# vedrocks15/Gradient-Based-Path-Tracing

Measured on AMD Instinct MI355X. Metric: GDPT Msamples/s (base+4 offset) + Poisson ms, cbox 512x512, higher is better.
Workload: dtype f64

## Files before the change

### gradient-based-path-tracing_amd/__init__.py

```python
import ctypes as C
import os

import numpy as np

from ._ctypes_defs import *
from . import _ctypes_defs as defs

_HERE = os.path.dirname(os.path.abspath(__file__))
LIB_PATH = os.path.join(_HERE, "libgdpt.so")
_LIB = None


class GdptError(RuntimeError):
    """Raised for a non-zero status from the C ABI (the reference throws fl_exception, src/flexception.h)."""


def library_path():
    return LIB_PATH


def lib():
    global _LIB
    if _LIB is None:
        if not os.path.exists(LIB_PATH):
# ... 7 lines not shown
        L.gdpt_parse_scene.argtypes = [C.c_char_p, C.POINTER(C.POINTER(defs.GdptSceneDesc))]
        L.gdpt_parse_scene_film.argtypes = [C.c_char_p, C.c_int, C.c_int, C.POINTER(C.POINTER(defs.GdptSceneDesc))]
        L.gdpt_free_scene_desc.argtypes = [C.POINTER(defs.GdptSceneDesc)]
        L.gdpt_scene_upload.argtypes = [C.POINTER(defs.GdptSceneDesc), C.c_int, C.POINTER(vp)]
        L.gdpt_scene_free.argtypes = [vp]
        L.gdpt_scene_info.argtypes = [vp] + [C.POINTER(C.c_int32)] * 4
        L.gdpt_render.argtypes = [vp, C.POINTER(defs.GdptRenderParams), dp, dp, dp, dp, dp, C.POINTER(defs.GdptRenderStats)]
        L.gdpt_render_device.argtypes = [vp, C.POINTER(defs.GdptRenderParams), vp, vp, vp, vp, vp, vp, C.POINTER(defs.GdptRenderStats)]
        L.gdpt_path_render.argtypes = [vp, C.POINTER(defs.GdptRenderParams), dp, C.POINTER(defs.GdptRenderStats)]
        L.gdpt_path_render_device.argtypes = [vp, C.POINTER(defs.GdptRenderParams), vp, vp, C.POINTER(defs.GdptRenderStats)]
        L.gdpt_render_window_device.argtypes = [vp, C.POINTER(defs.GdptRenderParams), C.POINTER(defs.GdptSampleWindow), vp, vp, vp, vp, vp, vp,
                                                C.POINTER(defs.GdptRenderStats)]
        L.gdpt_path_render_window_device.argtypes = [vp, C.POINTER(defs.GdptRenderParams), C.POINTER(defs.GdptSampleWindow), vp, vp,
                                                     C.POINTER(defs.GdptRenderStats)]
        L.gdpt_progressive_create.argtypes = [vp, C.POINTER(defs.GdptProgressiveConfig), vp, C.POINTER(vp)]
        L.gdpt_progressive_free.argtypes = [vp]
        L.gdpt_progressive_free.restype = None
        L.gdpt_progressive_add_pass.argtypes = [vp, C.c_int, C.POINTER(defs.GdptRenderStats)]
        L.gdpt_progressive_status.argtypes = [vp, C.POINTER(defs.GdptProgressiveStatus)]
        L.gdpt_progressive_read.argtypes = [vp, C.c_int, C.POINTER(vp), C.POINTER(vp), C.POINTER(vp)]
        L.gdpt_progressive_reconstruct.argtypes = [vp, C.c_double, C.POINTER(defs.GdptReconParams), C.c_int, vp, C.POINTER(defs.GdptReconStats)]
        L.gdpt_progressive_run.argtypes = [vp, C.c_double, C.c_int, C.c_int, C.POINTER(defs.GdptProgressiveStatus)]
        L.gdpt_progressive_create_slice.argtypes = [vp, C.POINTER(defs.GdptProgressiveConfig), C.c_int, C.c_int, vp, C.POINTER(vp)]
        L.gdpt_progressive_merge.argtypes = [vp, vp]
        L.gdpt_progressive_group_create.argtypes = [C.POINTER(defs.GdptSceneDesc), C.POINTER(C.c_int32), C.c_int,
                                                    C.POINTER(defs.GdptProgressiveConfig), C.POINTER(vp)]
        L.gdpt_progressive_group_free.argtypes = [vp]
        L.gdpt_progressive_group_free.restype = None
        L.gdpt_progressive_group_run.argtypes = [vp, C.c_double, C.c_int, C.c_int, C.POINTER(defs.GdptProgressiveStatus)]
        L.gdpt_progressive_group_total.argtypes = [vp]
        L.gdpt_progressive_group_total.restype = vp
        L.gdpt_progressive_group_member_status.argtypes = [vp, C.c_int, C.POINTER(defs.GdptProgressiveStatus)]
        sst, grp = C.POINTER(defs.GdptReconSpreadStats), C.POINTER(defs.GdptGroupReconParams)
        L.gdpt_recon_spread_device.argtypes = [C.c_int, C.c_int, C.c_int, C.POINTER(vp), dp, vp, C.c_int, vp, vp, vp, sst]
        L.gdpt_recon_spread.argtypes = [C.c_int, C.c_int, C.c_int, C.POINTER(vp), dp, vp, C.c_int, vp, vp, sst]
        L.gdpt_progressive_group_reconstruct_error.argtypes = [vp, grp, C.c_int, vp, vp, vp, sst, C.POINTER(defs.GdptReconStats)]
        L.gdpt_progressive_group_run_recon.argtypes = [vp, C.c_double, C.c_int, C.c_int, C.c_int, grp,
                                                       C.POINTER(defs.GdptProgressiveStatus), sst]
        L.gdpt_assemble_device.argtypes = [C.c_int, C.c_int, vp, vp, vp, vp, vp, vp, vp, vp, vp]
        L.gdpt_poisson_solve.argtypes = [C.c_int, C.c_int, dp, dp, dp, C.c_double, dp]
        L.gdpt_poisson_solve_ex.argtypes = [C.c_int, C.c_int, dp, dp, dp, C.c_double, dp, C.c_int, C.c_double, C.c_int,
                                            C.POINTER(defs.GdptPoissonStats)]
        L.gdpt_poisson_solve_device.argtypes = [C.c_int, C.c_int, vp, vp, vp, C.c_double, vp, C.c_int, C.c_double, C.c_int,
                                                vp, C.POINTER(defs.GdptPoissonStats)]
        L.gdpt_assemble_solve_device.argtypes = [C.c_int, C.c_int, vp, vp, vp, vp, vp, vp, vp, vp, C.c_double, vp, C.c_int, C.c_double, C.c_int,
                                                 vp, C.POINTER(defs.GdptPoissonStats)]
        L.gdpt_gradient_path_render.argtypes = [vp, C.POINTER(defs.GdptRenderParams), C.c_double, dp, dp, dp, dp, dp, dp,
                                                C.POINTER(defs.GdptRenderStats), C.POINTER(defs.GdptPoissonStats)]
        L.gdpt_reconstruct.argtypes = [C.c_int, C.c_int, dp, dp, dp, C.c_double, C.POINTER(defs.GdptReconParams), dp,
                                       C.POINTER(defs.GdptReconStats)]
        L.gdpt_reconstruct_device.argtypes = [C.c_int, C.c_int, vp, vp, vp, C.c_double, C.POINTER(defs.GdptReconParams), vp, vp,
                                              C.POINTER(defs.GdptReconStats)]
        L.gdpt_gradient_path_render_recon.argtypes = [vp, C.POINTER(defs.GdptRenderParams), C.c_double, C.POINTER(defs.GdptReconParams),
                                                      dp, dp, dp, dp, dp, dp, C.POINTER(defs.GdptRenderStats), C.POINTER(defs.GdptReconStats)]
        wp, wst = C.POINTER(defs.GdptWeightedReconParams), C.POINTER(defs.GdptWeightedReconStats)
        L.gdpt_reconstruct_weighted.argtypes = [C.c_int, C.c_int, dp, dp, dp, dp, dp, dp, C.c_double, wp, dp, C.POINTER(vp), wst]
        L.gdpt_reconstruct_weighted_device.argtypes = [C.c_int, C.c_int, vp, vp, vp, vp, vp, vp, C.c_double, wp, vp, C.POINTER(vp), vp, wst]
        L.gdpt_progressive_reconstruct_weighted.argtypes = [vp, C.c_double, wp, C.c_int, vp, C.POINTER(vp), wst]
        L.gdpt_imwrite.argtypes = [C.c_char_p, C.c_int, C.c_int, dp]
        L.gdpt_imread.argtypes = [C.c_char_p, C.c_int, C.POINTER(C.c_int), C.POINTER(C.c_int), C.POINTER(dp)]
        L.gdpt_image_free.argtypes = [dp]
        L.gdpt_bvh_check.argtypes = [C.POINTER(C.c_float), C.c_int, C.POINTER(C.c_int32)]
        L.gdpt_sbvh_check.argtypes = [C.POINTER(C.c_float), C.c_int, C.c_double, C.c_int, C.POINTER(C.c_int32)]
        L.gdpt_assemble_rows_device.argtypes = [C.c_int] * 4 + [vp] * 9
        L.gdpt_band_rows.argtypes = [C.c_int, C.c_int, C.c_int, C.POINTER(C.c_int32), C.POINTER(C.c_int32)]
        L.gdpt_band_rows_weighted.argtypes = [C.c_int, C.c_int, C.c_int, C.POINTER(C.c_double), C.c_int, C.POINTER(C.c_int32), C.POINTER(C.c_int32)]
        L.gdpt_tile_row_costs.argtypes = [vp, C.c_int, C.POINTER(C.c_double), C.c_int]
        L.gdpt_poisson_forget_stream.argtypes = [vp]
        L.gdpt_band_rows_from_row_costs.argtypes = [C.c_int, C.c_int, C.c_int, C.POINTER(C.c_double), C.c_int, C.POINTER(C.c_int32), C.POINTER(C.c_int32)]
        L.gdpt_multi_rebalance.argtypes = [vp, C.POINTER(C.c_double), C.c_int]
        L.gdpt_multi_create.argtypes = [C.POINTER(defs.GdptSceneDesc), C.POINTER(defs.GdptMultiConfig), C.POINTER(vp)]
        L.gdpt_multi_free.argtypes = [vp]
        L.gdpt_multi_free.restype = None
        L.gdpt_multi_gradient_path_render.argtypes = [vp, C.POINTER(defs.GdptRenderParams), C.c_double, dp, dp, dp, dp, dp, dp,
                                                      C.POINTER(defs.GdptRenderStats), C.POINTER(defs.GdptMultiStats)]
        L.gdpt_debug_knob_set.argtypes = [C.c_char_p, C.c_double]
        L.gdpt_debug_knobs_reset.restype = None
        L.gdpt_debug_chunk_plan.argtypes = [C.c_int, C.c_int, C.c_longlong, C.c_longlong, C.POINTER(C.c_int32), C.c_int]
        L.gdpt_debug_get_stamps.argtypes = [C.POINTER(C.c_double)]
        L.gdpt_debug_get_stamps.restype = None
        L.gdpt_debug_last_route.restype = C.c_char_p
        L.gdpt_debug_overlapped_launches.argtypes = [vp]
        L.gdpt_debug_overlapped_launches.restype = C.c_longlong
        L.gdpt_debug_route_names.argtypes = [C.POINTER(C.c_char_p), C.c_int]
        _LIB = L
    return _LIB


def _check(rc):
    if rc != 0:
        raise GdptError(lib().gdpt_last_error().decode("utf-8", "replace"))


def _dp(a):
    return a.ctypes.data_as(C.POINTER(C.c_double))


class SceneDesc:

    def __init__(self, ptr):
        self.ptr = ptr

    @property
    def desc(self):
        return self.ptr.contents

    @property
    def width(self):
        return self.ptr.contents.camera.width

    @property
    def height(self):
        return self.ptr.contents.camera.height

    def close(self):
        if self.ptr:
            lib().gdpt_free_scene_desc(self.ptr)
            self.ptr = None

    def __del__(self):
        try:
            self.close()
        except Exception:
            pass


def parse_scene(filename, film=(0, 0)):
    p = C.POINTER(defs.GdptSceneDesc)()
    _check(lib().gdpt_parse_scene_film(os.fsencode(filename), int(film[0]), int(film[1]), C.byref(p)))
    return SceneDesc(p)


def _params(spp, rng_scheme, rows, max_depth_override=0, shift=0, plan_rows=0):
    p = defs.GdptRenderParams()
    p.shift_mode = int(shift)
    p.plan_rows = int(plan_rows)
    p.spp, p.rng_scheme = int(spp), int(rng_scheme)
    p.row_begin, p.row_end = int(rows[0]), int(rows[1])
    p.max_depth_override = int(max_depth_override)
    return p


class Scene:

    def __init__(self, scene_desc, device=0):
        self.desc = scene_desc
        self.width, self.height = scene_desc.width, scene_desc.height
        h = C.c_void_p()
        _check(lib().gdpt_scene_upload(scene_desc.ptr, int(device), C.byref(h)))
        self.handle = h

    def info(self):
        v = [C.c_int32() for _ in range(4)]
        _check(lib().gdpt_scene_info(self.handle, *[C.byref(x) for x in v]))
        return dict(zip(("num_nodes", "num_tris", "num_spheres", "bvh_depth"), [x.value for x in v]))

    def render(self, spp=0, rng_scheme=defs.RNG_SAMPLE, rows=(0, 0), shift=defs.SHIFT_REFERENCE, plan_rows=0):
        shape = (self.height, self.width, 3)
        bufs = {k: np.zeros(shape, dtype=np.float64) for k in ("img", "cx0", "cy0", "cx1", "cy1")}
        st = defs.GdptRenderStats()
        p = _params(spp, rng_scheme, rows, shift=shift, plan_rows=plan_rows)
        _check(lib().gdpt_render(self.handle, C.byref(p), _dp(bufs["img"]), _dp(bufs["cx0"]), _dp(bufs["cy0"]),
                                 _dp(bufs["cx1"]), _dp(bufs["cy1"]), C.byref(st)))
        return bufs, st

    def render_device(self, ptrs, spp=0, rng_scheme=defs.RNG_SAMPLE, rows=(0, 0), stream=None, want_stats=False,
                      shift=defs.SHIFT_REFERENCE, plan_rows=0, window=None):
        st = defs.GdptRenderStats() if want_stats else None
        p = _params(spp, rng_scheme, rows, shift=shift, plan_rows=plan_rows)
        tail = [C.c_void_p(int(x)) for x in ptrs] + [C.c_void_p(int(stream) if stream else 0), C.byref(st) if st is not None else None]
        if window is None:
            _check(lib().gdpt_render_device(self.handle, C.byref(p), *tail))
        else:
            win = defs.GdptSampleWindow(int(window[0]), int(window[1]))
            _check(lib().gdpt_render_window_device(self.handle, C.byref(p), C.byref(win), *tail))
        return st

    def path_render(self, spp=0, rng_scheme=defs.RNG_SAMPLE, rows=(0, 0), want_counts=False):
        img = np.zeros((self.height, self.width, 3), dtype=np.float64)
        st = defs.GdptRenderStats()
        if want_counts:
            st.nodes_visited = 2 ** 64 - 1
        p = _params(spp, rng_scheme, rows)
        _check(lib().gdpt_path_render(self.handle, C.byref(p), _dp(img), C.byref(st)))
        return img, st

    def path_render_device(self, ptr, spp=0, rng_scheme=defs.RNG_SAMPLE, rows=(0, 0), stream=None, window=None, want_stats=False):
        st = defs.GdptRenderStats() if want_stats else None
        p = _params(spp, rng_scheme, rows)
        tail = [C.c_void_p(int(ptr)), C.c_void_p(int(stream) if stream else 0), C.byref(st) if st is not None else None]
        if window is None:
            _check(lib().gdpt_path_render_device(self.handle, C.byref(p), *tail))
        else:
            win = defs.GdptSampleWindow(int(window[0]), int(window[1]))
            _check(lib().gdpt_path_render_window_device(self.handle, C.byref(p), C.byref(win), *tail))
        return st

    def gradient_path_render(self, spp=0, rng_scheme=defs.RNG_SAMPLE, alpha=0.04, return_buffers=False,
                             shift=defs.SHIFT_REFERENCE, plan_rows=0, reconstruct=None):
        shape = (self.height, self.width, 3)
        out = np.zeros(shape, dtype=np.float64)
        bufs = {k: np.zeros(shape, dtype=np.float64) for k in ("img", "cx0", "cy0", "cx1", "cy1")}
        rs = defs.GdptRenderStats()
        p = _params(spp, rng_scheme, (0, 0), shift=shift, plan_rows=plan_rows)
        raw = [_dp(bufs[k]) for k in ("img", "cx0", "cy0", "cx1", "cy1")]
        if reconstruct is None:
            ps = defs.GdptPoissonStats()
            _check(lib().gdpt_gradient_path_render(self.handle, C.byref(p), float(alpha), _dp(out), *raw, C.byref(rs), C.byref(ps)))
        else:
            ps = defs.GdptReconStats()
            _check(lib().gdpt_gradient_path_render_recon(self.handle, C.byref(p), float(alpha), C.byref(reconstruct), _dp(out), *raw,
                                                         C.byref(rs), C.byref(ps)))
        return (out, bufs, rs, ps) if return_buffers else out

    def tile_row_costs(self, spp=1):
        T = (self.height + 15) // 16
        buf = (C.c_double * T)()
        _check(lib().gdpt_tile_row_costs(self.handle, int(spp), buf, T))
        return [float(x) for x in buf]

    def overlapped_launches(self):
        return int(lib().gdpt_debug_overlapped_launches(self.handle))

    def close(self):
        if getattr(self, "handle", None):
            lib().gdpt_scene_free(self.handle)
            self.handle = None

    def __del__(self):
        try:
            self.close()
        except Exception:
            pass


BUFFERS = ("img", "cx0", "cy0", "cx1", "cy1")


class Progressive:

    def __init__(self, scene, budget_spp, shift=defs.SHIFT_REFERENCE, path=False, stream=None, max_depth_override=0, slice=None):
        self.scene = scene
        self._owned = True
        self.path = bool(path)
        self.names = BUFFERS[:1] if self.path else BUFFERS
        self.shape = (scene.height, scene.width, 3)
        cfg = defs.GdptProgressiveConfig(defs.PROGRESSIVE_PATH if self.path else defs.PROGRESSIVE_GRADPATH, int(shift), int(budget_spp),
                                         int(max_depth_override))
        h = C.c_void_p()
        if slice is None:
            _check(lib().gdpt_progressive_create(scene.handle, C.byref(cfg), C.c_void_p(int(stream) if stream else 0), C.byref(h)))
        else:
            _check(lib().gdpt_progressive_create_slice(scene.handle, C.byref(cfg), int(slice[0]), int(slice[1]),
                                                       C.c_void_p(int(stream) if stream else 0), C.byref(h)))
        self.handle = h

    @classmethod
    def _view(cls, owner, handle, shape, path):
        self = cls.__new__(cls)
        self.scene, self._owned = owner, False
        self.path = bool(path)
        self.names = BUFFERS[:1] if self.path else BUFFERS
        self.shape = shape
        self.handle = C.c_void_p(handle)
        return self

    def merge(self, other):
        _check(lib().gdpt_progressive_merge(self.handle, other.handle))
        return self.status()

    def add_pass(self, spp):
        st = defs.GdptRenderStats()
        _check(lib().gdpt_progressive_add_pass(self.handle, int(spp), C.byref(st)))
        return st

    @staticmethod
    def _status_dict(st):
        return dict(passes=st.passes, spp=st.spp_done, budget_spp=st.budget_spp, error=st.error_estimate,
                    pixels_left_out=st.pixels_left_out, fold_ms=st.fold_ms, stop_reason=defs.STOP_NAMES[st.stop_reason], totals=st.totals)

    def status(self):
        st = defs.GdptProgressiveStatus()
        _check(lib().gdpt_progressive_status(self.handle, C.byref(st)))
        return self._status_dict(st)

    def read(self, variances=True):
        variances = bool(variances) and self.status()["passes"] >= 2
        means = {k: np.empty(self.shape, dtype=np.float64) for k in self.names}
        vars_ = {k: np.empty(self.shape, dtype=np.float64) for k in self.names} if variances else None
        asm = {k: np.empty(self.shape, dtype=np.float64) for k in ("c", "cx", "cy")} if variances and not self.path else None

        def table(d, keys):
            arr = (C.c_void_p * len(keys))()
            for i, k in enumerate(keys):
                arr[i] = d[k].ctypes.data if d is not None and k in d else None
            return arr
        _check(lib().gdpt_progressive_read(self.handle, 0, table(means, BUFFERS), table(vars_, BUFFERS), table(asm, ("c", "cx", "cy"))))
        return means, vars_, asm

    def read_device(self, mean_ptrs=None, var_ptrs=None, assembled_var_ptrs=None):
        def table(ptrs, n):
            arr = (C.c_void_p * n)()
            for i in range(n):
# ... 346 lines not shown
def shape_triangles(scene_desc):
    d = scene_desc.desc
    out = []
    for i in range(d.num_shapes):
        sh = d.shapes[i]
        if sh.num_triangles <= 0:
            continue
        pos = np.ctypeslib.as_array(sh.positions, shape=(sh.num_vertices, 3)).astype(np.float32)
        idx = np.ctypeslib.as_array(sh.indices, shape=(sh.num_triangles, 3))
        out.append(pos[idx])
    return np.concatenate(out, axis=0) if out else np.zeros((0, 3, 3), np.float32)


def shape_triangle_bounds(scene_desc):
    d = scene_desc.desc
    out = []
    for i in range(d.num_shapes):
        sh = d.shapes[i]
        if sh.num_triangles <= 0:
            continue
        pos = np.ctypeslib.as_array(sh.positions, shape=(sh.num_vertices, 3)).astype(np.float32)
        idx = np.ctypeslib.as_array(sh.indices, shape=(sh.num_triangles, 3))
        tri = pos[idx]
        out.append(np.concatenate([tri.min(axis=1), tri.max(axis=1)], axis=1))
    return np.concatenate(out, axis=0) if out else np.zeros((0, 6), np.float32)


class debug_knobs:

    def __init__(self, **knobs):
        self.knobs = knobs

    def __enter__(self):
        for k, v in self.knobs.items():
            _check(lib().gdpt_debug_knob_set(k.encode(), float(v)))
        return self

    def __exit__(self, *exc):
        lib().gdpt_debug_knobs_reset()
        return False

    @staticmethod
    def set(**knobs):
        for k, v in knobs.items():
            _check(lib().gdpt_debug_knob_set(k.encode(), float(v)))

    @staticmethod
    def reset():
        lib().gdpt_debug_knobs_reset()

    @staticmethod
    def chunk_plan(spp, film_pixels, resident_lanes=256 * 2 * 256, force_log2k=-1):
        buf = (C.c_int32 * 80)()
        n = lib().gdpt_debug_chunk_plan(int(spp), int(force_log2k), int(film_pixels), int(resident_lanes), buf, 80)
        if n < 0:
            raise GdptError("gdpt_debug_chunk_plan: capacity")
        return list(buf)[:n + 1]

    @staticmethod
    def stamps():
        v = (C.c_double * 16)()
        lib().gdpt_debug_get_stamps(v)
        d = dict(zip(("loop_head", "trace", "vertex", "consume", "bsdf", "finish", "camera", "wave_steps", "publish", "take", "item"), list(v)))
        d["busy_us"] = (v[13] - v[12]) / 100.0
        d["drain_us"] = (v[14] - v[13]) / 100.0
        return d

    @staticmethod
    def last_route():
        return lib().gdpt_debug_last_route().decode()

    @staticmethod
    def route_names():
        n = lib().gdpt_debug_route_names(None, 0)
        buf = (C.c_char_p * n)()
        if lib().gdpt_debug_route_names(buf, n) != n:
            raise GdptError("gdpt_debug_route_names: capacity")
        return [x.decode() for x in buf]

    @staticmethod
    def from_env(environ=None):
        environ = os.environ if environ is None else environ
        names = ("force_eager", "log2k", "keep_frac", "search_frac", "blocks_per_cu", "no_lds_scene", "lds_wide",
                 "no_twosided_machine", "presplit", "presplit_floor", "bvh_leaf_max", "bvh_leaf_factor", "sbvh", "sbvh_alpha", "plan_rounds", "plan_shrink", "plan_digits", "bvh_collapse_dp", "stamps", "wavefront", "wf_slots", "wf_sort", "multi_fail_band", "multi_fail_stage", "dct_bk", "dct_bm", "full_material_switch", "no_plain_kernel", "replay_per_step", "no_render_overlap")
        lib().gdpt_debug_knobs_reset()
        for n in names:
            v = environ.get("GDPT_" + n.upper())
            if v is not None:
                _check(lib().gdpt_debug_knob_set(n.encode(), float(v)))


def build_arch():
    return lib().gdpt_build_arch().decode()
```

### gradient-based-path-tracing_amd/csrc/capi_host.cpp

```cpp
#include "../../include/gdpt.h"
#include "../../include/gdpt_debug.h"
#include "capi_common.h"
#include "host/bvh.h"
#include "host/image_io.h"
#include "host/scene_loader.h"

#include <cmath>
#include <cstdlib>
#include <cstring>
#include <vector>
#include <algorithm>
#include <map>
#include <mutex>
#include <string>

namespace gdpt {
static thread_local std::string g_last_error;
void set_last_error(const std::string &msg) { g_last_error = msg; }
}

namespace gdpt {
namespace {
std::mutex g_knob_mu;
std::map<std::string, double> g_knobs;
const char *const kKnobNames[] = {"force_eager", "log2k", "keep_frac", "search_frac", "blocks_per_cu", "no_lds_scene", "lds_wide",
                                  "no_twosided_machine", "presplit", "presplit_floor", "bvh_leaf_max", "bvh_leaf_factor", "sbvh", "sbvh_alpha", "plan_rounds", "plan_shrink", "plan_digits", "bvh_collapse_dp", "stamps", "wavefront", "wf_slots", "wf_sort", "multi_fail_band", "multi_fail_stage", "dct_bk", "dct_bm", "full_material_switch", "no_plain_kernel", "replay_per_step", "no_render_overlap"};
double g_stamps[16] = {0};
}
void debug_store_stamps(const unsigned long long *v, int n) {
    std::lock_guard<std::mutex> lk(g_knob_mu);
    for (int i = 0; i < 16; i++) g_stamps[i] = i < n ? (double)v[i] : 0.0;
}
double debug_knob(const char *name, double def) {
    std::lock_guard<std::mutex> lk(g_knob_mu);
    if (g_knobs.empty()) return def;
    auto it = g_knobs.find(name);
    return it == g_knobs.end() ? def : it->second;
}
}

namespace {
std::mutex g_mu;
std::map<GdptSceneDesc *, std::unique_ptr<gdpt::HostScene>> g_descs;
}

extern "C" {

const char *gdpt_last_error(void) { return gdpt::g_last_error.c_str(); }

int gdpt_debug_knob_set(const char *name, double value) {
    return gdpt::guarded([&]() {
        if (!name) throw std::runtime_error("gdpt_debug_knob_set: null name");
        bool known = false;
        for (const char *k : gdpt::kKnobNames) if (std::strcmp(k, name) == 0) known = true;
        if (!known) throw std::runtime_error(std::string("gdpt_debug_knob_set: unknown knob '") + name + "'");
        std::lock_guard<std::mutex> lk(gdpt::g_knob_mu);
        gdpt::g_knobs[name] = value;
    });
}
void gdpt_debug_get_stamps(double out[16]) {
    std::lock_guard<std::mutex> lk(gdpt::g_knob_mu);
    for (int i = 0; i < 16; i++) out[i] = gdpt::g_stamps[i];
}
void gdpt_debug_knobs_reset(void) {
    std::lock_guard<std::mutex> lk(gdpt::g_knob_mu);
    gdpt::g_knobs.clear();
}

int gdpt_parse_scene(const char *xml_path, GdptSceneDesc **out_desc) { return gdpt_parse_scene_film(xml_path, 0, 0, out_desc); }

int gdpt_parse_scene_film(const char *xml_path, int film_width, int film_height, GdptSceneDesc **out_desc) {
    return gdpt::guarded([&]() {
        if (!xml_path || !out_desc) throw std::runtime_error("gdpt_parse_scene: null argument");
        if (film_width < 0 || film_height < 0 || film_width > 65536 || film_height > 65536) throw std::runtime_error("gdpt_parse_scene_film: bad film extent");
        std::unique_ptr<gdpt::HostScene> hs = gdpt::load_scene_xml(xml_path, film_width, film_height);
        GdptSceneDesc *d = &hs->desc;
        std::lock_guard<std::mutex> lk(g_mu);
        g_descs[d] = std::move(hs);
        *out_desc = d;
    });
}

void gdpt_free_scene_desc(GdptSceneDesc *desc) {
    std::lock_guard<std::mutex> lk(g_mu);
    g_descs.erase(desc);
}

int gdpt_imwrite(const char *filename, int width, int height, const double *rgb) {
    return gdpt::guarded([&]() {
        if (!filename || !rgb || width <= 0 || height <= 0) throw std::runtime_error("gdpt_imwrite: bad argument");
        gdpt::write_image(filename, width, height, rgb);
    });
}

int gdpt_imread(const char *filename, int channels, int *width, int *height, double **texels) {
    return gdpt::guarded([&]() {
        if (!filename || !width || !height || !texels || (channels != 1 && channels != 3)) throw std::runtime_error("gdpt_imread: bad argument");
        std::vector<double> t;
        gdpt::load_texture_file(filename, channels, width, height, &t);
        double *out = (double *)std::malloc(t.size() * sizeof(double));
        if (!out) throw std::runtime_error("gdpt_imread: out of memory");
        std::memcpy(out, t.data(), t.size() * sizeof(double));
        *texels = out;
    });
}

void gdpt_image_free(double *texels) { std::free(texels); }

int gdpt_sbvh_check(const float *tri_verts9, int n, double budget, int samples_per_tri, int32_t stats[8]) {
// ... 235 lines not shown
```

### gradient-based-path-tracing_amd/csrc/device_scene.h

```cpp
#pragma once
#include <stdint.h>

#define GDPT_BVH_MAX_DEPTH 32
#define GDPT_LEAF_MAX_PRIMS 4
#define GDPT_SPHERE_FLAG 0x80000000u
#ifndef GDPT_HBM_BVH8
#define GDPT_HBM_BVH8 0
#endif
#define GDPT_STACK_OVERFLOW 64
#ifndef GDPT_BVH8_SORT
#define GDPT_BVH8_SORT 1
#endif
#ifndef GDPT_SPEC_LEAF
#define GDPT_SPEC_LEAF 0
#endif
#define GDPT_CHILD_EMPTY INT32_MIN

struct DevBvhNode {
    float lmin[3], lmax[3];
    float rmin[3], rmax[3];
    int32_t left, right;
    int32_t pad[2];
};

struct DevBvh4Node {
    float lo[3][4];
    float hi[3][4];
    int32_t child[4];
    int32_t pad[4];
};

struct DevBvh8Node {
    int32_t child[8];
    uint8_t qlo[3][8];
    uint8_t qhi[3][8];
    float org[3];
    float scale[3];
    int32_t pad[6];
};

struct DevBvh4QNode {
    float org[3];
    float scale[3];
    uint8_t qlo[3][4];
    uint8_t qhi[3][4];
    int32_t child[4];
};
#ifndef GDPT_HBM_Q4
#define GDPT_HBM_Q4 1
#endif

struct DevPrim {
    float v0[3], e1[3], e2[3];
    uint32_t gid;
    uint32_t pad[2];
};

struct DevTriShade {
    double n[3][3];
    double uv[3][2];
    double dpdu[3], dpdv[3];
    double gn[3];
    double inv_uv_size;
    int32_t shape_id, prim_id, material_id, light_id;
    int32_t has_normals, has_uvs;
    int32_t flat_frame, pad;
};

struct DevSphere {
    double center[3];
    double radius;
    int32_t shape_id, material_id, light_id, pad;
};

struct DevLight {
    double intensity[3];
    double area;
    int32_t is_sphere;
    int32_t sphere_index;
    int32_t tri_first;
    int32_t tri_count;
    int32_t cdf_first;
    int32_t has_normals;
};

struct DevImage {
    int32_t channels, num_levels;
    int32_t width[8], height[8];
    int64_t offset[8];
};

struct DevCamera {
    double sample_to_cam[16];
    double cam_to_world[16];
    double org[3];
    int32_t width, height;
    int32_t filter_type;
    int32_t pow2_film;
    double filter_param;
    double inv_width, inv_height;
};

struct DevSceneView {
    DevCamera cam;
    const DevBvhNode *nodes;
    const DevBvh4Node *nodes4;
    const DevBvh8Node *nodes8;
    const DevBvh4QNode *nodes4q;
    const DevPrim *prims;
    const DevTriShade *tris;
    const DevSphere *spheres;
    const struct GdptMaterial *materials;
    const double *light_intensity;
    const DevImage *images;
    const double *texels;
    const DevLight *lights;
    const double *light_pmf, *light_cdf;
    const double *light_tri_cdf;
    const double *light_tri_pos;
    const double *light_tri_nrm;
    int32_t has_envmap, env_light_id, env_image_id, env_pad;
    int32_t env_w, env_h;
    double env_scale;
    double env_to_world[16], env_to_local[16];
    const double *env_cdf_rows, *env_pdf_rows, *env_cdf_marginals, *env_pdf_marginals;
    int32_t num_nodes, num_nodes4, num_nodes8, num_prims, num_tris, num_spheres;
    int32_t num_materials, num_lights, num_images;
    int32_t max_depth, rr_depth;
    int32_t all_textures_constant;
    double isect_eps;
};
```

### gradient-based-path-tracing_amd/csrc/hip/capi_device.hip

```cpp
#include "../../../include/gdpt.h"
#include "../capi_common.h"
#include "../device_scene.h"
#include "../host/bvh.h"
#include "../host/tri_precompute.h"
#include "poisson_kernels.h"
#include "recon_l1.h"
#include "recon_weighted.h"
#include "render_kernels.h"
#include "scene_internal.h"

#include <hip/hip_runtime.h>

#include <algorithm>
#include <cmath>
#include <cstdlib>
#include <cstring>
#include <limits>
#include <memory>
#include <string>
#include <vector>

namespace {

using gdpt::ck;
// ... 54 lines not shown
            for (int k = 0; k < 3; k++) { float p = (float)sh.positions[3 * i + k]; lb[k] = std::min(lb[k], p); ub[k] = std::max(ub[k], p); }
        for (int t = 0; t < sh.num_triangles; t++) {
            DevTriShade ts{};
            DevPrim pr{};
            gdpt::PrimBounds pb;
            float v[3][3];
            double pos64[3][3];
            for (int k = 0; k < 3; k++) { pb.bmin[k] = std::numeric_limits<float>::infinity(); pb.bmax[k] = -pb.bmin[k]; }
            for (int i = 0; i < 3; i++) {
                int vi = sh.indices[3 * t + i];
                if (vi < 0 || vi >= sh.num_vertices) throw std::runtime_error("gdpt_scene_upload: mesh index out of range");
                for (int k = 0; k < 3; k++) {
                    pos64[i][k] = sh.positions[3 * vi + k];
                    v[i][k] = (float)sh.positions[3 * vi + k];
                    pb.bmin[k] = std::min(pb.bmin[k], v[i][k]); pb.bmax[k] = std::max(pb.bmax[k], v[i][k]);
                    if (sh.normals) ts.n[i][k] = sh.normals[3 * vi + k];
                }
                if (sh.uvs) { ts.uv[i][0] = sh.uvs[2 * vi]; ts.uv[i][1] = sh.uvs[2 * vi + 1]; }
            }
            if (!sh.uvs) {
                ts.uv[0][0] = 0; ts.uv[0][1] = 0; ts.uv[1][0] = 1; ts.uv[1][1] = 0; ts.uv[2][0] = 1; ts.uv[2][1] = 1;
            }
            ts.shape_id = s; ts.prim_id = t; ts.material_id = sh.material_id; ts.light_id = sh.area_light_id;
            ts.has_normals = sh.normals != nullptr; ts.has_uvs = sh.uvs != nullptr;
            for (int k = 0; k < 3; k++) { pr.v0[k] = v[0][k]; pr.e1[k] = v[1][k] - v[0][k]; pr.e2[k] = v[2][k] - v[0][k]; }
            for (int i = 0; i < 3; i++) for (int k = 0; k < 3; k++) tri_verts.push_back(v[i][k]);
            gdpt::precompute_tri_constants(pos64, pr.e1, pr.e2, &ts);
            pr.gid = (uint32_t)tris.size();
            tris.push_back(ts); prim_in.push_back(pr); bounds.push_back(pb);
        }
    }
    if (tris.size() >= (size_t)GDPT_SPHERE_FLAG / 8) throw std::runtime_error("gdpt_scene_upload: too many triangles");
    for (int s = 0; s < desc->num_shapes; s++) {
        const GdptShape &sh = desc->shapes[s];
        if (sh.type != GDPT_SHAPE_SPHERE) continue;
        DevSphere sp{};
        DevPrim pr{};
        gdpt::PrimBounds pb;
        for (int k = 0; k < 3; k++) {
            sp.center[k] = sh.center[k];
            lb[k] = std::min(lb[k], (float)(sh.center[k] - sh.radius)); ub[k] = std::max(ub[k], (float)(sh.center[k] + sh.radius));
            pb.bmin[k] = std::nextafterf((float)(sh.center[k] - sh.radius), -std::numeric_limits<float>::infinity());
            pb.bmax[k] = std::nextafterf((float)(sh.center[k] + sh.radius), std::numeric_limits<float>::infinity());
        }
        sp.radius = sh.radius; sp.shape_id = s; sp.material_id = sh.material_id; sp.light_id = sh.area_light_id;
        pr.gid = GDPT_SPHERE_FLAG | (uint32_t)spheres.size();
        spheres.push_back(sp); prim_in.push_back(pr); bounds.push_back(pb);
    }

    std::vector<gdpt::PrimBounds> refs;
    std::vector<uint32_t> ref_prim;
    {
        double budget = tris.size() >= 4096 ? kPresplitBudget : 0.0;
        budget = gdpt::debug_knob("presplit", budget);
        gdpt::presplit_triangles(bounds, tri_verts, budget, &refs, &ref_prim);
    }
    const double sbvh_budget = gdpt::debug_knob("sbvh", tris.size() >= 4096 ? kSbvhBudget : 0.0);
    gdpt::BvhBuildResult bvh = sbvh_budget > 0 ? gdpt::build_sbvh(bounds, tri_verts, sbvh_budget, &ref_prim) : gdpt::build_bvh(refs);
    {
        float ext = 0.f;
        for (int k = 0; k < 3; k++) if (ub[k] >= lb[k]) ext = std::max(ext, std::max(std::fabs(ub[k]), std::fabs(lb[k])));
        for (auto &sp : spheres) for (int k = 0; k < 3; k++) ext = std::max(ext, (float)(std::fabs(sp.center[k]) + sp.radius));
        {
            const double *m = cam.cam_to_world;
            for (int k = 0; k < 3; k++) ext = std::max(ext, (float)std::fabs(m[4 * k + 3] / m[15]) * 1.0000002f);
        }
        const float pad = ext * 1e-6f + 1e-30f;
        for (auto &n : bvh.nodes)
            for (int k = 0; k < 3; k++) {
                if (n.lmin[k] <= n.lmax[k]) { n.lmin[k] -= pad; n.lmax[k] += pad; }
                if (n.rmin[k] <= n.rmax[k]) { n.rmin[k] -= pad; n.rmax[k] += pad; }
            }
    }
    gdpt::WideBvh wide = gdpt::collapse_for_traversal(bvh.nodes, GDPT_HBM_BVH8 != 0);
    if (wide.stack_need > GDPT_BVH_MAX_DEPTH) throw std::runtime_error("gdpt_scene_upload: BVH deeper than the traversal stack (builder bug)");
    if (wide.stack_need8 > GDPT_BVH_MAX_DEPTH + GDPT_STACK_OVERFLOW) throw std::runtime_error("gdpt_scene_upload: BVH8 deeper than the traversal stack (builder bug)");
    static_assert(sizeof(DevBvh8Node) == 128 && sizeof(DevBvh4Node) == 128, "wide BVH nodes are one 128-byte line");
    const std::vector<DevBvh4Node> &nodes4 = wide.nodes;
    sc->wide_stack_need = wide.stack_need;
    sc->wide8_stack_need = wide.stack_need8;
    std::vector<DevPrim> prims(bvh.order.size());
    for (size_t i = 0; i < bvh.order.size(); i++) prims[i] = prim_in[ref_prim[bvh.order[i]]];
    sc->bvh_depth = bvh.depth;
    if (bvh.depth > GDPT_BVH_MAX_DEPTH) throw std::runtime_error("gdpt_scene_upload: BVH deeper than the traversal stack (builder bug)");

    std::vector<DevImage> images;
    std::vector<double> texels;
    for (int i = 0; i < desc->num_images; i++) {
        const GdptImage &im = desc->images[i];
        if (im.width <= 0 || im.height <= 0 || (im.channels != 1 && im.channels != 3) || !im.texels)
            throw std::runtime_error("gdpt_scene_upload: bad image");
        DevImage di{};
        di.channels = im.channels;
        int size = std::max(im.width, im.height);
        int num_levels = std::min((int)std::ceil(std::log2((double)size) + 1), 8);
        di.num_levels = num_levels;
        int pw = im.width, ph = im.height;
        size_t prev_off = texels.size();
        di.width[0] = pw; di.height[0] = ph; di.offset[0] = (int64_t)prev_off;
        texels.insert(texels.end(), im.texels, im.texels + (size_t)pw * ph * im.channels);
        for (int l = 1; l < num_levels; l++) {
            int nw = std::max(pw / 2, 1), nh = std::max(ph / 2, 1);
            size_t off = texels.size();
            texels.resize(off + (size_t)nw * nh * im.channels);
            auto P = [&](int x, int y, int c) { x = std::min(x, pw - 1); y = std::min(y, ph - 1); return texels[prev_off + ((size_t)y * pw + x) * im.channels + c]; };
            for (int y = 0; y < nh; y++) for (int x = 0; x < nw; x++) for (int c = 0; c < im.channels; c++)
                texels[off + ((size_t)y * nw + x) * im.channels + c] =
                    (P(2 * x, 2 * y, c) + P(2 * x + 1, 2 * y, c) + P(2 * x, 2 * y + 1, c) + P(2 * x + 1, 2 * y + 1, c)) / 4.0;
            di.width[l] = nw; di.height[l] = nh; di.offset[l] = (int64_t)off;
            prev_off = off; pw = nw; ph = nh;
        }
        images.push_back(di);
    }

    std::vector<GdptMaterial> materials(desc->materials, desc->materials + desc->num_materials);
    std::vector<double> light_intensity;
    for (int l = 0; l < desc->num_lights; l++) for (int k = 0; k < 3; k++) light_intensity.push_back(desc->lights[l].intensity[k]);

    int env_power_slot = -1;
    std::vector<double> light_power;
    std::vector<DevLight> dlights;
    std::vector<double> light_pmf, light_cdf, light_tri_cdf, light_tri_pos, light_tri_nrm;
    auto table_1d = [](const std::vector<double> &f, std::vector<double> &pmf, std::vector<double> &cdf) {
        pmf = f;
        cdf.assign(f.size() + 1, 0.0);
        for (size_t i = 0; i < f.size(); i++) cdf[i + 1] = cdf[i] + pmf[i];
        const double total = cdf.back();
        if (total > 0) { for (size_t i = 0; i < pmf.size(); i++) { pmf[i] /= total; cdf[i] /= total; } }
        else {
            for (size_t i = 0; i < pmf.size(); i++) { pmf[i] = 1.0 / (double)pmf.size(); cdf[i] = (double)i / (double)pmf.size(); }
            cdf.back() = 1;
        }
    };
    {
        std::vector<int> sphere_index_of_shape((size_t)desc->num_shapes, -1);
        { int k = 0; for (int s = 0; s < desc->num_shapes; s++) if (desc->shapes[s].type == GDPT_SHAPE_SPHERE) sphere_index_of_shape[(size_t)s] = k++; }
        std::vector<double> power;
        for (int l = 0; l < desc->num_lights; l++) {
            const GdptLight &lt = desc->lights[l];
            if (lt.shape_id < 0 && desc->has_envmap && l == desc->envmap.light_id) {
                dlights.push_back(DevLight{});
                power.push_back(0.0);
                continue;
            }
            if (lt.shape_id < 0 || lt.shape_id >= desc->num_shapes) throw std::runtime_error("gdpt_scene_upload: light without a shape");
            const GdptShape &sh = desc->shapes[lt.shape_id];
            DevLight dl{};
            for (int k = 0; k < 3; k++) dl.intensity[k] = lt.intensity[k];
            if (sh.type == GDPT_SHAPE_SPHERE) {
                dl.is_sphere = 1; dl.sphere_index = sphere_index_of_shape[(size_t)lt.shape_id];
                dl.area = 4 * 3.14159265358979323846 * sh.radius * sh.radius;
            } else {
                dl.tri_first = (int)(light_tri_pos.size() / 9); dl.tri_count = sh.num_triangles;
                dl.cdf_first = (int)light_tri_cdf.size(); dl.has_normals = sh.normals ? 1 : 0;
                std::vector<double> areas((size_t)sh.num_triangles), pmf, cdf;
                double total = 0;
                for (int t = 0; t < sh.num_triangles; t++) {
                    const int *ix = sh.indices + 3 * t;
                    double p[3][3];
                    for (int i = 0; i < 3; i++) for (int k = 0; k < 3; k++) { p[i][k] = sh.positions[3 * ix[i] + k]; light_tri_pos.push_back(p[i][k]); }
                    for (int i = 0; i < 3; i++) for (int k = 0; k < 3; k++) light_tri_nrm.push_back(sh.normals ? sh.normals[3 * ix[i] + k] : 0.0);
                    const double e1[3] = {p[1][0] - p[0][0], p[1][1] - p[0][1], p[1][2] - p[0][2]}, e2[3] = {p[2][0] - p[0][0], p[2][1] - p[0][1], p[2][2] - p[0][2]};
                    const double cx = e1[1] * e2[2] - e1[2] * e2[1], cy = e1[2] * e2[0] - e1[0] * e2[2], cz = e1[0] * e2[1] - e1[1] * e2[0];
                    areas[(size_t)t] = std::sqrt(cx * cx + cy * cy + cz * cz) / 2;
                    total += areas[(size_t)t];
                }
// ... 160 lines not shown

Band resolve_spp(const GdptScene *sc, const GdptRenderParams *p, int scene_spp, const char *what, const GdptSampleWindow *win = nullptr) {
    Band b = resolve(sc, p);
    if (b.spp <= 0) b.spp = scene_spp;
    if (b.spp <= 0) throw std::runtime_error(std::string(what) + ": samples per pixel must be > 0");
    b.stream_spp = b.spp; b.first_sample = 0;
    if (win) {
        if (b.rng == GDPT_RNG_TILE) throw std::runtime_error(std::string(what) + ": GDPT_RNG_TILE has one stream per tile and no sample window (use GDPT_RNG_SAMPLE)");
        if (win->stream_spp <= 0 || win->first_sample < 0 || (long long)win->first_sample + b.spp > (long long)win->stream_spp)
            throw std::runtime_error(std::string(what) + ": sample window [first_sample, first_sample + spp) must lie inside [0, stream_spp)");
        if ((unsigned long long)sc->view.cam.width * (unsigned long long)sc->view.cam.height > (~0ull >> 1) / (unsigned long long)win->stream_spp)
            throw std::runtime_error(std::string(what) + ": width * height * stream_spp does not fit 63 bits");
        b.stream_spp = win->stream_spp; b.first_sample = win->first_sample;
    }
    return b;
}

struct ScratchClaim { GdptLaunchScratch *set = nullptr; bool record_release = true; };

bool is_capturing(hipStream_t stream) {
    hipStreamCaptureStatus st = hipStreamCaptureStatusNone;
    if (hipStreamIsCapturing(stream, &st) != hipSuccess) { (void)hipGetLastError(); return true; }
    return st != hipStreamCaptureStatusNone;
}

void join_scratch(GdptScene *sc) {
    sc->join();
    for (auto &ss : sc->scratch) if (ss.used) ck(hipEventSynchronize(ss.released), "hipEventSynchronize(launch scratch)");
}

GdptLaunchScratch &claim_scratch(GdptScene *sc, bool overlap, bool capturing, size_t need, hipStream_t stream) {
    const int k = overlap ? (int)(sc->overlapped & 1) : 0;
    GdptLaunchScratch &ss = sc->scratch[k];
    const hipEvent_t entry = sc->ev_entry[sc->calls & 1], prev_entry = sc->calls ? (hipEvent_t)sc->ev_entry[(sc->calls + 1) & 1] : nullptr;
    if (!capturing) { ck(hipEventRecord(entry, stream), "hipEventRecord(entry)"); sc->calls++; }
    if (capturing) {
        hipStreamCaptureMode mode = hipStreamCaptureModeRelaxed;
        ck(hipThreadExchangeStreamCaptureMode(&mode), "hipThreadExchangeStreamCaptureMode");
        try { join_scratch(sc); } catch (...) { (void)hipThreadExchangeStreamCaptureMode(&mode); throw; }
        ck(hipThreadExchangeStreamCaptureMode(&mode), "hipThreadExchangeStreamCaptureMode");
    }
    if (!ss.counters) ss.counters.alloc(1, "hipMalloc(counters)");
    if (!ss.queue) ss.queue.alloc(1, "hipMalloc(queue)");
    if (need > ss.partials.size()) {
        if (ss.partials) {
            if (!capturing) join_scratch(sc);
            sc->need_fence = true;
        }
        ss.partials.alloc(need, "hipMalloc(work-item partials)");
    }
    if (!overlap) {
        if (!capturing) {
            sc->join();
            if (ss.used) ck(hipStreamWaitEvent(stream, ss.released, 0), "hipStreamWaitEvent(launch scratch)");
        }
    } else {
        if (sc->have_caller && stream != sc->last_caller) {
            for (auto &o : sc->scratch) ck(hipStreamWaitEvent(stream, o.rendered, 0), "hipStreamWaitEvent(render stream)");
            sc->need_fence = true;
        }
        if (sc->need_fence || !prev_entry) {
            for (auto &st : sc->render_stream) ck(hipStreamWaitEvent(st, entry, 0), "hipStreamWaitEvent(fence)");
            sc->need_fence = false;
        } else
            ck(hipStreamWaitEvent(sc->render_stream[k], prev_entry, 0), "hipStreamWaitEvent(previous call)");
        if (ss.used) ck(hipStreamWaitEvent(sc->render_stream[k], ss.released, 0), "hipStreamWaitEvent(launch scratch)");
    }
    sc->have_caller = true; sc->last_caller = stream;
    return ss;
}

gdpt::RenderLaunch begin_launch(GdptScene *sc, const Band &b, bool path, int take_pct, hipStream_t stream, const GdptRenderStats *stats, ScratchClaim *claim) {
    auto knob = [](const char *name, int def) { return gdpt::debug_knob_int(name, def); };
    const DevSceneView &v = sc->view;
    gdpt::RouteInputs in{};
    in.path = path; in.rng_scheme = b.rng; in.shift_mode = b.shift; in.max_depth = b.max_depth; in.rr_depth = v.rr_depth;
    in.one_sided = sc->one_sided; in.has_rough = sc->has_rough; in.lambert_only = sc->lambert_only; in.material_mask = sc->material_mask;
    in.has_spheres = v.num_spheres != 0; in.const_textures = v.all_textures_constant != 0; in.has_envmap = v.has_envmap != 0;
    in.fits_lds = gdpt::scene_fits_lds(v.num_nodes, v.num_prims, v.num_tris, v.num_materials, v.num_lights, sc->bvh_depth);
    in.fits_lds_wide = gdpt::scene_fits_lds_wide(v.num_nodes4, v.num_prims, v.num_tris, v.num_materials, v.num_lights, sc->wide_stack_need);
    in.force_eager = knob("force_eager", 0) != 0; in.no_lds_scene = knob("no_lds_scene", 0) != 0; in.lds_wide = knob("lds_wide", 1) != 0;
    in.no_twosided_machine = knob("no_twosided_machine", 0) != 0; in.wavefront = knob("wavefront", kWavefrontDefault) != 0;
    in.stamps = knob("stamps", 0) != 0; in.no_plain_kernel = knob("no_plain_kernel", 0) != 0;
    in.full_material_switch = knob("full_material_switch", 0) != 0;
    gdpt::RenderLaunch rl{};
    rl.route = gdpt::choose_route(in);
    rl.spp = b.spp; rl.stream_spp = b.stream_spp; rl.first_sample = b.first_sample; rl.row_begin = b.row_begin; rl.row_end = b.row_end; rl.max_depth = b.max_depth;
    rl.count_traversal = stats && stats->nodes_visited == ~0ull;
    rl.force_log2k = knob("log2k", -1);
    rl.thresh_a = knob("keep_frac", -1); rl.thresh_c = knob("search_frac", -1);
    rl.num_cus = sc->num_cus; rl.blocks_per_cu = knob("blocks_per_cu", 0);
    const bool capturing = is_capturing(stream);
    const bool overlap = !stats && gdpt::can_overlap(rl.route) && !capturing && knob("no_render_overlap", 0) == 0;
    size_t need = 0;
    if (gdpt::is_persistent(rl.route)) {
        rl.plan = gdpt::make_chunk_plan(b.spp, rl.force_log2k, (long long)v.cam.width * b.plan_rows, gdpt::resident_lanes(rl), take_pct);
        need = (size_t)16 * (size_t)gdpt::band_slots(v.cam.width, b.row_end - b.row_begin) * (size_t)rl.plan.n;
    }
    GdptLaunchScratch &ss = claim_scratch(sc, overlap, capturing, need, stream);
    rl.counters = ss.counters; sc->d_counters = ss.counters;
    if (gdpt::is_persistent(rl.route)) { rl.partials = ss.partials; rl.queue_head = ss.queue; }
    if (overlap) { rl.kernel_stream = sc->render_stream[sc->overlapped & 1]; rl.kernel_done = ss.rendered; }
    claim->set = &ss; claim->record_release = !capturing;
    return rl;
}

void run_launch(GdptScene *sc, const gdpt::RenderLaunch &rl, const ScratchClaim &claim, const Band &b, hipStream_t stream, GdptRenderStats *stats) {
    const bool stamped = gdpt::is_stamped(rl.route);
    const hipStream_t ks = rl.kernel_stream ? rl.kernel_stream : stream;
    if (rl.kernel_stream) sc->in_flight = true;
    ck(hipMemsetAsync(rl.counters, 0, sizeof(gdpt::RenderCounters), ks), "hipMemsetAsync(counters)");
    if (stamped) ck(hipMemsetAsync(&rl.counters->stamps[12], 0xFF, 2 * sizeof(unsigned long long), ks), "hipMemsetAsync(stamps)");
    if (stats) ck(hipEventRecord(sc->ev0, stream), "hipEventRecord");
    gdpt::launch_render(sc->view, rl, stream);
    if (rl.kernel_stream) sc->overlapped++;
    if (claim.record_release) { ck(hipEventRecord(claim.set->released, stream), "hipEventRecord(launch scratch)"); claim.set->used = true; }
    if (!stats) return;
    ck(hipEventRecord(sc->ev1, stream), "hipEventRecord");
    ck(hipMemcpyAsync(sc->h_counters, rl.counters, sizeof(gdpt::RenderCounters), hipMemcpyDeviceToHost, stream), "hipMemcpyAsync(counters)");
    ck(hipStreamSynchronize(stream), "hipStreamSynchronize(render)");
    float ms = 0;
    ck(hipEventElapsedTime(&ms, sc->ev0, sc->ev1), "hipEventElapsedTime");
    const gdpt::RenderCounters &c = *sc->h_counters;
    std::memset(stats, 0, sizeof(*stats));
    stats->samples = (uint64_t)sc->view.cam.width * (uint64_t)(b.row_end - b.row_begin) * (uint64_t)b.spp;
    stats->rays = c.rays; stats->bounces = c.bounces; stats->nonfinite_samples = c.nonfinite;
    stats->nodes_visited = c.nodes; stats->tris_tested = c.prims;
    stats->render_ms = ms;
    if (!gdpt::is_path(rl.route)) {
        stats->wave_node_trips = c.wave_node_trips; stats->wave_leaf_trips = c.wave_leaf_trips;
        stats->wave_steps = c.wave_steps; stats->lane_steps = c.lane_steps;
    }
    if (stamped) gdpt::debug_store_stamps(c.stamps, 16);
    stats->node_bytes = gdpt::walks_bvh2(rl.route) ? sizeof(DevBvhNode) : sizeof(DevBvh4Node);
}

}

namespace gdpt {
void render_device_impl(GdptScene *sc, const GdptRenderParams *params, int scene_spp,
                        double *img, double *cx0, double *cy0, double *cx1, double *cy1,
                        hipStream_t stream, GdptRenderStats *stats, const GdptSampleWindow *window) {
    reset_route();
    ck(hipSetDevice(sc->device), "hipSetDevice");
    const Band b = resolve_spp(sc, params, scene_spp, "gdpt_render", window);
    if (!img || !cx0 || !cy0 || !cx1 || !cy1) throw std::runtime_error("gdpt_render: null output buffer");
    ScratchClaim claim;
    RenderLaunch rl = begin_launch(sc, b, false, sc->plan_take_pct, stream, stats, &claim);
    rl.img = img; rl.cx0 = cx0; rl.cy0 = cy0; rl.cx1 = cx1; rl.cy1 = cy1;
    rl.wide_stack_need = GDPT_HBM_BVH8 ? std::min(sc->wide8_stack_need, GDPT_BVH_MAX_DEPTH) : sc->wide_stack_need;
    rl.replay_per_step = debug_knob_int("replay_per_step", 0);
    const long long items = band_slots(sc->view.cam.width, b.row_end - b.row_begin) * rl.plan.n;
    if (needs_bounce_log(rl.route)) {
        sc->d_bounce_log.grow(twosided_log_bytes(persistent_blocks(rl, items)), stream, "hipMalloc(bounce log)");
        rl.bounce_log = sc->d_bounce_log; rl.bounce_log_bytes = sc->d_bounce_log.size();
    }
    if (is_wavefront(rl.route)) {
        int slots = wf_slot_count(items);
        { const int forced = debug_knob_int("wf_slots", 0); if (forced > 0) slots = std::min(slots, (forced + 255) / 256 * 256); }
        sc->d_wf_state.grow((size_t)slots * wf_words(), stream, "hipMalloc(wavefront state)");
        sc->d_wf_live.grow((size_t)slots, stream, "hipMalloc(wavefront live list)");
        sc->d_wf_aux.grow(wf_aux_bytes(slots), stream, "hipMalloc(wavefront ray / hit records)");
        if (!sc->d_wf_counters) sc->d_wf_counters.alloc((size_t)3 * wf_max_generations(), "hipMalloc(wavefront counters)");
        if (!sc->h_wf_word) sc->h_wf_word.alloc(1, "hipHostMalloc(wavefront)");
        if (!sc->wf_event) sc->wf_event.create(hipEventDisableTiming);
        rl.wf_aux = sc->d_wf_aux; rl.wf_sort = debug_knob_int("wf_sort", 1);
        for (int k = 0; k < 6; k++) rl.wf_bounds[k] = sc->bounds[k];
        rl.wf_state = sc->d_wf_state; rl.wf_live = sc->d_wf_live; rl.wf_counters = sc->d_wf_counters; rl.wf_host = sc->h_wf_word;
        rl.wf_event = sc->wf_event; rl.wf_slots = slots;
// ... 17 lines not shown
    rl.img = img;
    run_launch(sc, rl, claim, b, stream, stats);
}

gdpt::ReconL1Params resolve_recon(const GdptReconParams &in) {
    if (in.norm != GDPT_RECON_L1) throw std::runtime_error("gdpt_reconstruct: unknown norm (GDPT_RECON_L2 | GDPT_RECON_L1)");
    for (double v : {in.eps_init, in.eps_decay, in.eps_floor, in.cg_tol})
        if (!std::isfinite(v) || v < 0) throw std::runtime_error("gdpt_reconstruct: eps_init, eps_decay, eps_floor and cg_tol must be finite and >= 0 (0 = default)");
    if (in.eps_decay > 1.0) throw std::runtime_error("gdpt_reconstruct: eps_decay must lie in (0, 1]");
    gdpt::ReconL1Params p;
    p.irls_iters = in.irls_iters == 0 ? 20 : std::max(in.irls_iters, 0);
    p.cg_max_iters = in.cg_max_iters > 0 ? in.cg_max_iters : 1000;
    p.eps_init = in.eps_init > 0 ? in.eps_init : 0.05;
    p.eps_decay = in.eps_decay > 0 ? in.eps_decay : 0.5;
    p.eps_floor = in.eps_floor > 0 ? in.eps_floor : 1e-3;
    p.cg_tol = in.cg_tol > 0 ? in.cg_tol : 1e-6;
    return p;
}
using Planes = std::vector<gdpt::DeviceBuffer<double>>;
template <class F>
void on_device_planes(std::initializer_list<const double *> in, int width, int height, double *out, const char *what, F &&run) {
    const size_t elems = (size_t)width * height * 3, bytes = elems * sizeof(double);
    Planes d(in.size() + 1);
    for (auto &b : d) b.alloc(elems, what);
    size_t k = 0;
    for (const double *h : in) ck(hipMemcpy(d[k++], h, bytes, hipMemcpyHostToDevice), "hipMemcpy");
    run(d);
    ck(hipMemcpy(out, d.back(), bytes, hipMemcpyDeviceToHost), "hipMemcpy");
}

void fill_poisson_stats(GdptPoissonStats *s, const gdpt::PoissonResult &r) {
    if (!s) return;
    s->iterations = r.iterations; s->solver = r.solver; s->rel_residual = r.rel_residual; s->solve_ms = r.solve_ms;
}
void fill_recon_stats(GdptReconStats *s, const gdpt::ReconL1Result &r) {
    if (!s) return;
    s->norm = GDPT_RECON_L1; s->irls_rounds = r.irls_rounds; s->cg_iters_total = r.cg_iters_total; s->cg_iters_last = r.cg_iters_last;
    s->energy_first = r.energy_first; s->energy_last = r.energy_last; s->rel_residual_last = r.rel_residual_last; s->solve_ms = r.solve_ms;
}
void fill_recon_stats_l2(GdptReconStats *s, double solve_ms) {
    if (!s) return;
    *s = GdptReconStats{};
    s->norm = GDPT_RECON_L2; s->solve_ms = solve_ms;
}

gdpt::ReconL1Params resolve_weighted(const GdptWeightedReconParams *in, double *conf_floor, int *norm) {
    GdptReconParams rp = in ? in->recon : GdptReconParams{};
    *norm = rp.norm;
    if (rp.norm != GDPT_RECON_L2 && rp.norm != GDPT_RECON_L1) throw std::runtime_error("gdpt_reconstruct_weighted: unknown norm (GDPT_RECON_L2 | GDPT_RECON_L1)");
    rp.norm = GDPT_RECON_L1;
    gdpt::ReconL1Params p = resolve_recon(rp);
    if (*norm == GDPT_RECON_L2) p.irls_iters = 0;
    const double d = in ? in->conf_floor : 0.0;
    if (!std::isfinite(d) || d < 0) throw std::runtime_error("gdpt_reconstruct_weighted: conf_floor must be finite and > 0 (0 = default 0.05)");
    *conf_floor = d > 0 ? d : 0.05;
    return p;
}
void fill_weighted_stats(GdptWeightedReconStats *s, int norm, const gdpt::ReconWeightedResult &r) {
    if (!s) return;
    *s = GdptWeightedReconStats{};
    fill_recon_stats(&s->recon, r.recon);
    s->recon.norm = norm;
    s->scale_data = r.scale_data; s->scale_grad = r.scale_grad; s->rows_dropped = r.rows_dropped; s->pixels_isolated = r.pixels_isolated;
}

}

extern "C" {

#ifndef GDPT_BUILD_ARCH
#error "GDPT_BUILD_ARCH must name the --offload-arch the kernels were compiled for (csrc/Makefile passes it)"
#endif
const char *gdpt_build_arch(void) { return GDPT_BUILD_ARCH; }

int gdpt_debug_chunk_plan(int spp, int force_log2k, long long film_pixels, long long resident_lanes, int32_t *begin, int capacity) {
    const gdpt::ChunkPlan p = gdpt::make_chunk_plan(spp, force_log2k, film_pixels, resident_lanes);
    if (!begin || capacity < p.n + 1) return -1;
    for (int c = 0; c <= p.n; c++) begin[c] = p.begin[c];
    return p.n;
}

const char *gdpt_debug_last_route(void) { return gdpt::last_route(); }
long long gdpt_debug_overlapped_launches(const GdptScene *scene) { return scene ? (long long)scene->overlapped : -1; }
int gdpt_debug_route_names(const char **out, int capacity) { return gdpt::route_names(out, capacity); }

int gdpt_scene_upload(const GdptSceneDesc *desc, int device, GdptScene **out_scene) {
    return gdpt::guarded([&]() {
        if (!out_scene) throw std::runtime_error("gdpt_scene_upload: null output");
        std::unique_ptr<GdptScene> sc(new GdptScene());
        build_scene(desc, device, sc.get());
        sc->scene_spp = desc->samples_per_pixel;
        *out_scene = sc.release();
    });
}

void gdpt_scene_free(GdptScene *scene) {
    if (!scene) return;
    delete scene;
}

int gdpt_scene_info(const GdptScene *scene, int32_t *num_nodes, int32_t *num_tris, int32_t *num_spheres, int32_t *bvh_depth) {
    return gdpt::guarded([&]() {
        if (!scene) throw std::runtime_error("null scene handle");
        if (num_nodes) *num_nodes = scene->view.num_nodes;
        if (num_tris) *num_tris = scene->view.num_tris;
        if (num_spheres) *num_spheres = scene->view.num_spheres;
        if (bvh_depth) *bvh_depth = scene->bvh_depth;
    });
}

int gdpt_render_device(GdptScene *scene, const GdptRenderParams *params,
                       double *d_img, double *d_cx0, double *d_cy0, double *d_cx1, double *d_cy1,
                       void *stream, GdptRenderStats *stats) {
    return gdpt::guarded([&]() {
        if (!scene) throw std::runtime_error("null scene handle");
        render_device_impl(scene, params, scene->scene_spp, d_img, d_cx0, d_cy0, d_cx1, d_cy1, (hipStream_t)stream, stats);
    });
}

int gdpt_render(GdptScene *scene, const GdptRenderParams *params,
                double *img, double *cx0, double *cy0, double *cx1, double *cy1, GdptRenderStats *stats) {
    return gdpt::guarded([&]() {
        if (!scene) throw std::runtime_error("null scene handle");
        if (!img || !cx0 || !cy0 || !cx1 || !cy1) throw std::runtime_error("gdpt_render: null output buffer");
        ck(hipSetDevice(scene->device), "hipSetDevice");
        size_t elems = (size_t)scene->view.cam.width * scene->view.cam.height * 3;
        scene->ensure_buffers(elems);
        Band b = resolve(scene, params);
        double *host[5] = {img, cx0, cy0, cx1, cy1};
        bool partial = (b.row_begin != 0 || b.row_end != scene->view.cam.height);
        if (partial) for (int k = 0; k < 5; k++) ck(hipMemcpy(scene->d_buf[k], host[k], elems * sizeof(double), hipMemcpyHostToDevice), "hipMemcpy(H2D)");
        GdptRenderStats local{};
        render_device_impl(scene, params, scene->scene_spp, scene->d_buf[0], scene->d_buf[1], scene->d_buf[2], scene->d_buf[3], scene->d_buf[4],
                           nullptr, stats ? stats : &local);
        for (int k = 0; k < 5; k++) ck(hipMemcpy(host[k], scene->d_buf[k], elems * sizeof(double), hipMemcpyDeviceToHost), "hipMemcpy(D2H)");
    });
}

int gdpt_tile_row_costs(GdptScene *scene, int spp, double *cost, int capacity) {
    return gdpt::guarded([&]() {
        if (!scene || !cost) throw std::runtime_error("gdpt_tile_row_costs: null argument");
        const int H = scene->view.cam.height, T = (H + 15) / 16;
        if (capacity < T) throw std::runtime_error("gdpt_tile_row_costs: capacity < ceil(height / 16)");
        ck(hipSetDevice(scene->device), "hipSetDevice");
        scene->ensure_buffers((size_t)scene->view.cam.width * H * 3);
        for (int t = 0; t < T; t++) {
            GdptRenderParams p{};
            p.spp = spp > 0 ? spp : 1; p.rng_scheme = GDPT_RNG_SAMPLE; p.row_begin = t * 16; p.row_end = std::min(H, t * 16 + 16);
            GdptRenderStats st{};
            render_device_impl(scene, &p, scene->scene_spp, scene->d_buf[0], scene->d_buf[1], scene->d_buf[2], scene->d_buf[3], scene->d_buf[4], nullptr, &st);
            cost[t] = (double)st.rays;
        }
    });
}

int gdpt_path_render_device(GdptScene *scene, const GdptRenderParams *params, double *d_img, void *stream, GdptRenderStats *stats) {
    return gdpt::guarded([&]() {
        if (!scene) throw std::runtime_error("null scene handle");
        path_render_device_impl(scene, params, d_img, (hipStream_t)stream, stats, nullptr);
    });
}

int gdpt_render_window_device(GdptScene *scene, const GdptRenderParams *params, const GdptSampleWindow *window,
                              double *d_img, double *d_cx0, double *d_cy0, double *d_cx1, double *d_cy1,
                              void *stream, GdptRenderStats *stats) {
    if (!window) return gdpt_render_device(scene, params, d_img, d_cx0, d_cy0, d_cx1, d_cy1, stream, stats);
// ... 217 lines not shown
```

### gradient-based-path-tracing_amd/csrc/hip/render_device.h

```cpp
#pragma once
#include "render_kernels.h"
#include "device_trace.h"

namespace gd {

constexpr int kBlock = 256;
constexpr int kLdsSceneBytes = 20 * 1024;
constexpr int kLdsSceneLevels = 12;

struct LaneCounters { unsigned rays, bounces, nonfinite; };

enum { SEG_QUEUE = 0, SEG_TRACE = 1, SEG_VERTEX = 2, SEG_CONSUME = 3, SEG_BSDF = 4, SEG_FINISH = 5, SEG_CAMERA = 6, SEG_STEPS = 7, SEG_PUBLISH = 8, SEG_TAKE = 9, SEG_ITEM = 10, SEG_COUNT = 12, SEG_T_START = 12, SEG_T_DRY = 13, SEG_T_END = 14, SEG_SLOTS = 16 };
template <bool ON> struct Stamps {
    unsigned long long *slot;
    GD void start(unsigned long long *wave_row) {
        if (ON) { slot = wave_row; if ((threadIdx.x & 63) == 0) { for (int i = 0; i < SEG_COUNT; i++) slot[i] = 0; slot[SEG_COUNT] = __builtin_amdgcn_s_memtime(); } }
    }
    GD void mark(int seg) {
        if (ON) {
            __builtin_amdgcn_sched_barrier(0);
            const unsigned long long t = __builtin_amdgcn_s_memtime();
            __builtin_amdgcn_s_waitcnt(0xC07F);
            if ((int)(threadIdx.x & 63) == __ffsll((unsigned long long)__ballot(1)) - 1) { slot[seg] += t - slot[SEG_COUNT]; slot[SEG_COUNT] = t; }
            __builtin_amdgcn_sched_barrier(0);
        }
    }
    GD void tick(int seg) { if (ON) { if ((int)(threadIdx.x & 63) == __ffsll((unsigned long long)__ballot(1)) - 1) slot[seg] += 1; } }
    GD unsigned long long get(int seg) const { return ON ? slot[seg] : 0ull; }
};
struct Accum { D3 r, dx0, dy0, dx1, dy1; };

struct KernelArgs {
    int spp, log2k, tile_w, tile_h, tiles_x;
    int row_begin, row_end, max_depth;
    int thresh_a, thresh_c;
    int count;
    int stream_spp, first_sample;
    int stack_levels;
    int replay_per_step;
    int num_chunks;
    long long num_slots;
    long long num_items;
    double *partials;
    int chunk_begin[gdpt::kMaxChunks + 1];
    unsigned long long *queue_head;
    double *img, *cx0, *cy0, *cx1, *cy1;
    gdpt::RenderCounters *counters;
};

GD bool loop_allows(int max_depth, int num_vertices) { return max_depth == -1 || num_vertices <= max_depth + 1; }

struct AccReg {
    Accum a;
    GD void init() { a.r = a.dx0 = a.dy0 = a.dx1 = a.dy1 = splat(0); }
    GD void add(int which, D3 v) {
        if (which == 0) a.r = a.r + v; else if (which == 1) a.dx0 = a.dx0 + v; else if (which == 2) a.dy0 = a.dy0 + v;
        else if (which == 3) a.dx1 = a.dx1 + v; else a.dy1 = a.dy1 + v;
    }
    GD Accum result() { return a; }
};
struct AccLds {
    double *slot;
    int stride;
    GD void init() { for (int c = 0; c < 15; c++) slot[c * stride] = 0.0; }
    GD void add(int which, D3 v) {
        double *p = slot + which * 3 * stride;
        __hip_atomic_fetch_add(p, v.x, __ATOMIC_RELAXED, __HIP_MEMORY_SCOPE_WORKGROUP);
        __hip_atomic_fetch_add(p + stride, v.y, __ATOMIC_RELAXED, __HIP_MEMORY_SCOPE_WORKGROUP);
        __hip_atomic_fetch_add(p + 2 * stride, v.z, __ATOMIC_RELAXED, __HIP_MEMORY_SCOPE_WORKGROUP);
    }
    GD Accum result() {
        Accum a;
        a.r = mk(slot[0], slot[stride], slot[2 * stride]);
        a.dx0 = mk(slot[3 * stride], slot[4 * stride], slot[5 * stride]);
        a.dy0 = mk(slot[6 * stride], slot[7 * stride], slot[8 * stride]);
        a.dx1 = mk(slot[9 * stride], slot[10 * stride], slot[11 * stride]);
        a.dy1 = mk(slot[12 * stride], slot[13 * stride], slot[14 * stride]);
        return a;
    }
};

template <class ACC>
GD void acc_base(ACC &a, D3 radiance, double prob, double spp, LaneCounters &lc, bool counted = false) {
    if (!counted && !(isfinite(prob) && isfinite(radiance.x + radiance.y + radiance.z))) lc.nonfinite++;
    if (prob > 0.0) a.add(0, radiance / spp);
// ... 99 lines not shown
#pragma unroll
        for (int k = 0; k < 3; k++) {
            const float qa = (float)((nq[k] >> (8 * c)) & 0xffu), qb = (float)((fq[k] >> (8 * c)) & 0xffu);
            t0 = fmaxf(t0, fmaf(qa, A[k], B[k])); t1 = fminf(t1, fmaf(qb, A[k], B[k]));
        }
        const int ch = c == 0 ? c0 : (c == 1 ? c1 : (c == 2 ? c2 : c3));
        const bool h = (ch != GDPT_CHILD_EMPTY) && (t0 <= t1);
        w.key[c] = h ? ((__float_as_uint(t0) & ~3u) | (unsigned)c) : kMissKey;
    }
#define GDPT_CSWAP(i, j) { unsigned lo_ = min(w.key[i], w.key[j]), hi_ = max(w.key[i], w.key[j]); w.key[i] = lo_; w.key[j] = hi_; }
    GDPT_CSWAP(0, 1) GDPT_CSWAP(2, 3) GDPT_CSWAP(0, 2) GDPT_CSWAP(1, 3) GDPT_CSWAP(1, 2)
#undef GDPT_CSWAP
#pragma unroll
    for (int i = 0; i < 4; i++) w.ch[i] = pick4(w.key[i], c0, c1, c2, c3);
}

struct Wide8Visit { unsigned key[8]; };
GD int pick8(unsigned k, const int c[8]) {
    const int a0 = (k & 1u) ? c[1] : c[0], a1 = (k & 1u) ? c[3] : c[2], a2 = (k & 1u) ? c[5] : c[4], a3 = (k & 1u) ? c[7] : c[6];
    const int b0 = (k & 2u) ? a1 : a0, b1 = (k & 2u) ? a3 : a2;
    return (k & 4u) ? b1 : b0;
}
GD void visit_wide8(const DevBvh8Node &n, const float oi[3], const float inv[3], float tnear, float tb, int ch[8], Wide8Visit &w) {
    const uint4 *qp = (const uint4 *)&n.qlo[0][0];
    const uint4 q0 = qp[0], q1 = qp[1], q2 = qp[2];
    const unsigned lo[3][2] = {{q0.x, q0.y}, {q0.z, q0.w}, {q1.x, q1.y}};
    const unsigned hi[3][2] = {{q1.z, q1.w}, {q2.x, q2.y}, {q2.z, q2.w}};
    float A[3], B[3];
    unsigned nq[3][2], fq[3][2];
#pragma unroll
    for (int k = 0; k < 3; k++) {
        A[k] = n.scale[k] * inv[k];
        B[k] = fmaf(n.org[k], inv[k], -oi[k]);
        const bool neg = inv[k] < 0.0f;
#pragma unroll
        for (int h = 0; h < 2; h++) { nq[k][h] = neg ? hi[k][h] : lo[k][h]; fq[k][h] = neg ? lo[k][h] : hi[k][h]; }
    }
#pragma unroll
    for (int c = 0; c < 8; c++) ch[c] = n.child[c];
#pragma unroll
    for (int c = 0; c < 8; c++) {
        float t0 = tnear, t1 = tb;
#pragma unroll
        for (int k = 0; k < 3; k++) {
            const float qa = (float)((nq[k][c >> 2] >> (8 * (c & 3))) & 0xffu), qb = (float)((fq[k][c >> 2] >> (8 * (c & 3))) & 0xffu);
            t0 = fmaxf(t0, fmaf(qa, A[k], B[k])); t1 = fminf(t1, fmaf(qb, A[k], B[k]));
        }
        const bool h = (ch[c] != GDPT_CHILD_EMPTY) && (t0 <= t1);
        w.key[c] = h ? ((__float_as_uint(t0) & ~7u) | (unsigned)c) : kMissKey;
    }
    if (!GDPT_BVH8_SORT) return;
#define GDPT_CSWAP(i, j) { unsigned lo_ = min(w.key[i], w.key[j]), hi_ = max(w.key[i], w.key[j]); w.key[i] = lo_; w.key[j] = hi_; }
    GDPT_CSWAP(0, 1) GDPT_CSWAP(2, 3) GDPT_CSWAP(4, 5) GDPT_CSWAP(6, 7)
    GDPT_CSWAP(0, 2) GDPT_CSWAP(1, 3) GDPT_CSWAP(4, 6) GDPT_CSWAP(5, 7)
    GDPT_CSWAP(1, 2) GDPT_CSWAP(5, 6) GDPT_CSWAP(0, 4) GDPT_CSWAP(3, 7)
    GDPT_CSWAP(1, 5) GDPT_CSWAP(2, 6)
    GDPT_CSWAP(1, 4) GDPT_CSWAP(3, 6)
    GDPT_CSWAP(2, 4) GDPT_CSWAP(3, 5)
    GDPT_CSWAP(3, 4)
#undef GDPT_CSWAP
}

template <bool FLAT, bool SPHERES = true>
GD void test_leaf(const DevSceneView &sv, const TraceCtx &tx, int cur, const float o[3], const float d[3], float tnear, float tfar,
                  Hit &best, TraceCounters &tc) {
    const unsigned packed = ~(unsigned)cur;
    const unsigned first = packed >> 2, last = packed & 3u;
    const DevPrim p0 = tx.prims[first];
    const DevPrim p1 = tx.prims[first + min(1u, last)];
    const DevPrim p2 = tx.prims[first + min(2u, last)];
    const DevPrim p3 = tx.prims[first + last];
    if (tx.count) { tc.prims += last + 1u; if (wave_leader()) tc.leaf_trips++; }
    if (!FLAT || (SPHERES && ((p0.gid | p1.gid | p2.gid | p3.gid) & GDPT_SPHERE_FLAG))) {
        test_prim<SPHERES>(sv, p0, o, d, tnear, tfar, best);
        if (last >= 1u) test_prim<SPHERES>(sv, p1, o, d, tnear, tfar, best);
        if (last >= 2u) test_prim<SPHERES>(sv, p2, o, d, tnear, tfar, best);
        if (last >= 3u) test_prim<SPHERES>(sv, p3, o, d, tnear, tfar, best);
    } else {
        test_tri_flat(p0, o, d, tnear, tfar, true, best);
        test_tri_flat(p1, o, d, tnear, tfar, last >= 1u, best);
        test_tri_flat(p2, o, d, tnear, tfar, last >= 2u, best);
        test_tri_flat(p3, o, d, tnear, tfar, last >= 3u, best);
    }
}

constexpr int kTravDone = INT32_MIN;
struct Trav { Hit best; int cur, sp; int ovf[GDPT_STACK_OVERFLOW]; };
GD void trav_init(const DevSceneView &sv, Trav &tv, double tfar) {
    tv.best.gid = -1; tv.best.t = (float)tfar; tv.best.u = tv.best.v = 0; tv.best.ngx = tv.best.ngy = tv.best.ngz = 0;
    tv.sp = 0; tv.cur = (sv.num_nodes == 0) ? kTravDone : 0;
}
template <bool OVF = false>
GD void trav_pop(const TraceCtx &tx, int &cur, int &sp, int *ovf = nullptr) {
    if (sp > 0) {
        sp--;
        if (OVF && sp >= GDPT_BVH_MAX_DEPTH) cur = ovf[sp - GDPT_BVH_MAX_DEPTH];
        else cur = tx.stack[sp * tx.stride];
    } else cur = kTravDone;
}
template <bool OVF = false>
GD void trav_push(const TraceCtx &tx, int &sp, int x, int *ovf = nullptr) {
    if (OVF && sp >= GDPT_BVH_MAX_DEPTH) ovf[sp - GDPT_BVH_MAX_DEPTH] = x;
    else tx.stack[sp * tx.stride] = x;
    sp++;
}
template <bool WIDE, bool HBM = false>
GD void trav_node(const TraceCtx &tx, const float oi[3], const float inv[3], float tnear, float tb, int &cur, int &sp, int *ovf) {
    if (WIDE && HBM && GDPT_HBM_BVH8) {
        Wide8Visit w;
        int ch[8];
        visit_wide8(tx.nodes8[cur], oi, inv, tnear, tb, ch, w);
        if (GDPT_BVH8_SORT) {
            if (w.key[0] != kMissKey) {
#pragma unroll
                for (int i = 7; i >= 1; i--) if (w.key[i] != kMissKey) trav_push<true>(tx, sp, pick8(w.key[i], ch), ovf);
                cur = pick8(w.key[0], ch);
            } else trav_pop<true>(tx, cur, sp, ovf);
        } else {
            unsigned near = w.key[0];
#pragma unroll
            for (int c = 1; c < 8; c++) near = min(near, w.key[c]);
            if (near != kMissKey) {
#pragma unroll
                for (int c = 0; c < 8; c++) if (w.key[c] != kMissKey && w.key[c] != near) trav_push<true>(tx, sp, ch[c], ovf);
                cur = pick8(near, ch);
            } else trav_pop<true>(tx, cur, sp, ovf);
        }
    } else if (WIDE) {
        WideVisit w;
#ifdef GDPT_EXTRA_LOOKUPS
        if (HBM) {
            const char *np = (const char *)&tx.nodes4[cur];
            unsigned d0, d1, d2, d3, d4, d5, d6;
            asm volatile("global_load_dword %0, %7, off\n global_load_dword %1, %7, off offset:16\n global_load_dword %2, %7, off offset:32\n"
                         "global_load_dword %3, %7, off offset:48\n global_load_dword %4, %7, off offset:64\n global_load_dword %5, %7, off offset:80\n"
                         "global_load_dword %6, %7, off offset:96\n s_waitcnt vmcnt(0)"
                         : "=&v"(d0), "=&v"(d1), "=&v"(d2), "=&v"(d3), "=&v"(d4), "=&v"(d5), "=&v"(d6) : "v"(np) : "memory");
        }
#endif
        if (HBM && GDPT_HBM_Q4) visit_wide_q4(tx.nodes4q[cur], oi, inv, tnear, tb, w);
        else visit_wide<!HBM>(tx.nodes4[cur], oi, inv, tnear, tb, w);
        if (w.key[0] != kMissKey) {
            if (w.key[3] != kMissKey) trav_push(tx, sp, w.ch[3]);
            if (w.key[2] != kMissKey) trav_push(tx, sp, w.ch[2]);
            if (w.key[1] != kMissKey) trav_push(tx, sp, w.ch[1]);
            cur = w.ch[0];
        } else trav_pop(tx, cur, sp);
    } else {
        const DevBvhNode &n = tx.nodes[cur];
        float tl, tr;
        bool hl = (n.left != GDPT_CHILD_EMPTY) && box_hit(n.lmin, n.lmax, oi, inv, tnear, tb, tl);
        bool hr = (n.right != GDPT_CHILD_EMPTY) && box_hit(n.rmin, n.rmax, oi, inv, tnear, tb, tr);
        if (hl && hr) {
            int nearc = n.left, farc = n.right;
            if (tr < tl) { nearc = n.right; farc = n.left; }
            trav_push(tx, sp, farc);
            cur = nearc;
        } else if (hl) cur = n.left;
        else if (hr) cur = n.right;
        else trav_pop(tx, cur, sp);
    }
}
template <bool WW_, bool WIDE_, bool FLAT_, bool SPHERES_ = true, bool SPEC_ = false> struct TraceCfg { static constexpr bool WW = WW_, WIDE = WIDE_, FLAT = FLAT_, SPHERES = SPHERES_, SPEC = SPEC_ || GDPT_SPEC_LEAF; };
using TraceHbm = TraceCfg<true, true, true>;

template <class TC>
GD void trav_run(const DevSceneView &sv, const TraceCtx &tx, D3 org, D3 dir, float tnear, float tfar, Trav &tv, int stop_below, int search_frac, TraceCounters &tc,
                 bool any_hit = false) {
    const float o[3] = {(float)org.x, (float)org.y, (float)org.z};
    const float d[3] = {(float)dir.x, (float)dir.y, (float)dir.z};
    float inv[3] = {1.0f / d[0], 1.0f / d[1], 1.0f / d[2]};
    float oi[3] = {o[0] * inv[0], o[1] * inv[1], o[2] * inv[2]};
#pragma unroll
    for (int k = 0; k < 3; k++) if (d[k] == 0.0f) { inv[k] = __builtin_nanf(""); oi[k] = __builtin_nanf(""); }
    constexpr bool kOvf = TC::WIDE && TC::FLAT && GDPT_HBM_BVH8;
    int cur = tv.cur, sp = tv.sp;
    Hit best = tv.best;
    for (;;) {
        const int live = __popcll(__ballot(cur != kTravDone));
        if (live <= stop_below) break;
        if (TC::WW) {
            const int few = (live * search_frac) >> 8;
            if (TC::SPEC) {
                int held = kTravDone;
                for (;;) {
                    if (cur < 0 && cur != kTravDone && held == kTravDone) { held = cur; trav_pop<kOvf>(tx, cur, sp, tv.ovf); }
                    const bool searching = cur >= 0;
                    if (__popcll(__ballot(searching)) <= few) break;
                    if (searching) {
                        if (tx.count) { tc.nodes++; if (wave_leader()) tc.node_trips++; }
                        trav_node<TC::WIDE, TC::FLAT>(tx, oi, inv, tnear, best.t, cur, sp, tv.ovf);
                    }
                }
                if (held != kTravDone) {
                    test_leaf<TC::FLAT, TC::SPHERES>(sv, tx, held, o, d, tnear, tfar, best, tc);
                    if (any_hit && best.gid >= 0) cur = kTravDone;
                }
            } else {
                for (;;) {
                    const bool searching = cur >= 0;
                    if (__popcll(__ballot(searching)) <= few) break;
                    if (searching) {
                        if (tx.count) { tc.nodes++; if (wave_leader()) tc.node_trips++; }
                        trav_node<TC::WIDE, TC::FLAT>(tx, oi, inv, tnear, best.t, cur, sp, tv.ovf);
                    }
                }
                if (cur < 0 && cur != kTravDone) {
                    test_leaf<TC::FLAT, TC::SPHERES>(sv, tx, cur, o, d, tnear, tfar, best, tc);
                    trav_pop<kOvf>(tx, cur, sp, tv.ovf);
                    if (any_hit && best.gid >= 0) cur = kTravDone;
                }
            }
        } else if (cur >= 0) {
            if (tx.count) { tc.nodes++; if (wave_leader()) tc.node_trips++; }
            trav_node<TC::WIDE, TC::FLAT>(tx, oi, inv, tnear, best.t, cur, sp, tv.ovf);
        } else if (cur != kTravDone) {
            test_leaf<TC::FLAT, TC::SPHERES>(sv, tx, cur, o, d, tnear, tfar, best, tc);
            trav_pop<kOvf>(tx, cur, sp, tv.ovf);
            if (any_hit && best.gid >= 0) cur = kTravDone;
        }
    }
    tv.cur = cur; tv.sp = sp; tv.best = best;
}

constexpr int kEagerSearchFrac = 112;

template <class TC>
GD bool intersect_ctx(const DevSceneView &sv, const TraceCtx &tx, const Ray &ray, double rd_spread, Vertex &v, LaneCounters &lc, TraceCounters &tc) {
    lc.rays++;
    Trav tv;
    trav_init(sv, tv, ray.tfar);
    if (tv.cur != kTravDone) trav_run<TC>(sv, tx, ray.org, ray.dir, (float)ray.tnear, (float)ray.tfar, tv, 0, kEagerSearchFrac, tc);
    if (tv.best.gid < 0) return false;
    make_vertex(sv, tx.tris, tx.need_uv, ray, tv.best, 0.0, rd_spread, v);
    return true;
}

template <class TC>
GD bool occluded_ctx(const DevSceneView &sv, const TraceCtx &tx, const Ray &ray, LaneCounters &lc, TraceCounters &tc) {
    lc.rays++;
    Trav tv;
    trav_init(sv, tv, ray.tfar);
    if (tv.cur != kTravDone) trav_run<TC>(sv, tx, ray.org, ray.dir, (float)ray.tnear, (float)ray.tfar, tv, 0, kEagerSearchFrac, tc, true);
    return tv.best.gid >= 0;
}

template <bool LAMBERT, bool ROUGH = false, bool TWOSIDED = false, unsigned MASK = kAllMaterials>
GD bool mat_sample(const DevSceneView &sv, const TraceCtx &tx, const Vertex &v, D3 in, D2 ruv, double rw, BsdfSample &s) {
    if (LAMBERT) { Ctx c{sv, v}; return cos_sample(c, in, ruv, 1.0, s); }
    return bsdf_sample<ROUGH, TWOSIDED, MASK>(sv, tx.materials[v.material_id], in, v, ruv, rw, s);
}
template <bool LAMBERT, bool ROUGH = false, bool TWOSIDED = false, unsigned MASK = kAllMaterials, int PLAIN = 0>
GD void mat_eval_pdf(const DevSceneView &sv, const TraceCtx &tx, const Vertex &v, D3 in, D3 out, D3 &f, double &pdf) {
    if (LAMBERT) {
        if (below(v, in) || below(v, out)) { f = splat(0); pdf = 0; return; }
        Frame fr = oriented_frame(v, in);
        double c = fmax(dot(fr.n, out), 0.0);
        const GdptTexture &refl = tx.materials[v.material_id].tex[0];
        f = c * ((PLAIN & kPlainConstTex) ? mk(refl.v0[0], refl.v0[1], refl.v0[2]) : tex3(sv, refl, v)) / kPi;
        pdf = c / kPi;
        return;
    }
    const GdptMaterial &m = tx.materials[v.material_id];
    bsdf_eval_pdf<ROUGH, TWOSIDED, MASK>(sv, m, in, out, v, f, pdf);
}
template <bool LAMBERT>
GD double mat_pdf(const DevSceneView &sv, const TraceCtx &tx, const Vertex &v, D3 in, D3 out) {
    if (LAMBERT) { Ctx c{sv, v}; return cos_pdf(c, in, out); }
    return bsdf_pdf(sv, tx.materials[v.material_id], in, out, v);
}

enum { S_START = 0, S_PRIMARY = 1, S_BOUNCE = 2, S_OFFSET = 3, S_DONE = 4 };
enum { ACT_NONE = 0, ACT_BOUNCE = 1, ACT_OFFSETS = 2, ACT_NEXT_SAMPLE = 3, ACT_PRIMARY_RAY = 4, ACT_OFFSET_RAY = 5 };
enum { C_NO_LOOP = 0,
       C_AFTER_BOUNCE1 = 1,
       C_BROKE_BOUNCE1 = 2,
       C_BROKE_BOUNCE2 = 3 };

struct LanePriv {
    double *slot; int stride;
    GD D3 radiance() const { return mk(slot[0], slot[stride], slot[2 * stride]); }
    GD void set_radiance(D3 v) { slot[0] = v.x; slot[stride] = v.y; slot[2 * stride] = v.z; }
    GD double p2_1() const { return slot[3 * stride]; }
    GD void set_p2_1(double v) { slot[3 * stride] = v; }
    GD FilterCache fc() const { FilterCache f; f.dx = slot[4 * stride]; f.dy = slot[5 * stride]; f.ox = slot[6 * stride]; f.oy = slot[7 * stride]; return f; }
    GD void set_fc(const FilterCache &f) { slot[4 * stride] = f.dx; slot[5 * stride] = f.dy; slot[6 * stride] = f.ox; slot[7 * stride] = f.oy; }
};
constexpr int kPrivDoubles = 8;

constexpr int kKcNonfinite = 1 << 30;
struct Lane {
    int st, s, s_end, num_vertices;
    int mats;
    int kc;
    unsigned long long rng_state, rng_inc;
    D3 org, dir;
    D3 f; double pdf;
    D3 contrib, throughput;
    double prob;
    double rng_x, rng_y;
    D2 ruv1; double rw1;
// ... 232 lines not shown
        a.img[i] = acc.r.x; a.img[i + 1] = acc.r.y; a.img[i + 2] = acc.r.z;
        a.cx0[i] = acc.dx0.x; a.cx0[i + 1] = acc.dx0.y; a.cx0[i + 2] = acc.dx0.z;
        a.cy0[i] = acc.dy0.x; a.cy0[i + 1] = acc.dy0.y; a.cy0[i + 2] = acc.dy0.z;
        a.cx1[i] = acc.dx1.x; a.cx1[i + 1] = acc.dx1.y; a.cx1[i + 2] = acc.dx1.z;
        a.cy1[i] = acc.dy1.x; a.cy1[i + 1] = acc.dy1.y; a.cy1[i + 2] = acc.dy1.z;
    }
}

inline size_t hbm_dynamic_lds(const KernelArgs &a) { return (size_t)a.stack_levels * kBlock * sizeof(int); }

template <bool LDS_SCENE, bool WIDE>
GD TraceCtx setup_trace(const DevSceneView &sv, unsigned char *s_scene, int *s_stack, int tid, int nthreads, bool count) {
    TraceCtx tx;
    tx.count = count;
    tx.need_uv = !sv.all_textures_constant;
    tx.stack = s_stack + tid; tx.stride = nthreads;
    if (LDS_SCENE) {
        const int nw = WIDE ? sv.num_nodes4 * (int)(sizeof(DevBvh4Node) / 4) : sv.num_nodes * (int)(sizeof(DevBvhNode) / 4);
        const int pw = sv.num_prims * (int)(sizeof(DevPrim) / 4);
        const int tw = sv.num_tris * (int)(sizeof(DevTriShade) / 4), mw = sv.num_materials * (int)(sizeof(GdptMaterial) / 4);
        unsigned *dst = (unsigned *)s_scene;
        const unsigned *s0 = WIDE ? (const unsigned *)sv.nodes4 : (const unsigned *)sv.nodes;
        const unsigned *s1 = (const unsigned *)sv.prims, *s2 = (const unsigned *)sv.tris, *s3 = (const unsigned *)sv.materials;
        for (int i = tid; i < nw; i += nthreads) dst[i] = s0[i];
        for (int i = tid; i < pw; i += nthreads) dst[nw + i] = s1[i];
        for (int i = tid; i < tw; i += nthreads) dst[nw + pw + i] = s2[i];
        for (int i = tid; i < mw; i += nthreads) dst[nw + pw + tw + i] = s3[i];
        const int l0 = (nw + pw + tw + mw + 1) & ~1, lw = sv.num_lights * 6;
        const unsigned *s4 = (const unsigned *)sv.light_intensity;
        for (int i = tid; i < lw; i += nthreads) dst[l0 + i] = s4[i];
        __syncthreads();
        tx.lights = (const double *)(s_scene + (size_t)l0 * 4);
        tx.nodes = (const DevBvhNode *)s_scene; tx.nodes4 = (const DevBvh4Node *)s_scene; tx.nodes8 = nullptr; tx.nodes4q = nullptr;
        tx.prims = (const DevPrim *)(s_scene + (size_t)nw * 4);
        tx.tris = (const DevTriShade *)(s_scene + (size_t)(nw + pw) * 4);
        tx.materials = (const GdptMaterial *)(s_scene + (size_t)(nw + pw + tw) * 4);
    } else {
        tx.nodes = sv.nodes; tx.nodes4 = sv.nodes4; tx.nodes8 = sv.nodes8; tx.nodes4q = sv.nodes4q; tx.prims = sv.prims; tx.tris = sv.tris; tx.materials = sv.materials;
        tx.lights = sv.light_intensity;
    }
    return tx;
}

GD bool item_to_pixel(const KernelArgs &a, int W, unsigned item, int &x, int &y, int &s0, int &s1, const int *chunks) {
    const unsigned c = item / (unsigned)a.num_slots, pt = item - c * (unsigned)a.num_slots;
    const unsigned pin = pt & 255u, tile = pt >> 8;
    const unsigned ty = tile / (unsigned)a.tiles_x, tx = tile - ty * (unsigned)a.tiles_x;
    x = (int)(tx * 16u + (pin & 15u)); y = a.row_begin + (int)(ty * 16u + (pin >> 4));
    s0 = chunks[c]; s1 = chunks[c + 1];
    return x < W && y < a.row_end;
}

struct WaveQueue {
    long long next = 0, end = 0, seen_head = 0;
    bool exhausted = false;
    GD long long take(const KernelArgs &a, bool idle, int tid) {
        long long item = -1;
        const unsigned long long m_idle = __ballot(idle);
        if (m_idle) {
            if (next >= end && !exhausted) {
                const unsigned left = (unsigned)(a.num_items - seen_head);
                const unsigned waves = gridDim.x * (unsigned)(kBlock / 64);
                const long long n_idle_now = __popcll(m_idle);
                long long want = 64;
                if (left < waves * 64u) { want = (long long)(left / (waves * 2u)); want = want > 64 ? 64 : (want < n_idle_now ? n_idle_now : want); }
                unsigned long long got = 0;
                if ((tid & 63) == 0) got = atomicAdd(a.queue_head, (unsigned long long)want);
                got = __shfl(got, 0, 64);
                next = (long long)got;
                end = min((long long)got + want, a.num_items);
                seen_head = end;
                if (next >= a.num_items) { exhausted = true; end = next; }
            }
            const int avail = (int)(end - next);
            const int rank = __popcll(m_idle & ((1ull << (tid & 63)) - 1ull));
            if (idle && rank < avail) item = next + rank;
            const int n_idle = __popcll(m_idle);
            next += (n_idle < avail) ? n_idle : avail;
        }
        return item;
    }
};

template <bool LAMBERT, bool LDS_SCENE, bool WIDE, bool WW, bool STAMPED = false, int PLAIN = 0>
__global__ __launch_bounds__(kBlock, 2) void gdpt_render_phases(DevSceneView sv, KernelArgs a) {
    __shared__ int s_stack_fixed[LDS_SCENE ? kLdsSceneLevels * kBlock : 1];
    __shared__ __attribute__((aligned(16))) unsigned char s_scene[LDS_SCENE ? kLdsSceneBytes : 16];
    __shared__ double s_acc[15 * kBlock];
    __shared__ double s_priv[kPrivDoubles * kBlock];
    __shared__ int s_chunks[66];
    extern __shared__ __attribute__((aligned(16))) unsigned char s_dyn[];
    int *s_stack = LDS_SCENE ? s_stack_fixed : (int *)s_dyn;
    const int tid = threadIdx.x;
    if (tid <= a.num_chunks && tid < 66) s_chunks[tid] = a.chunk_begin[tid];
    TraceCtx tx = setup_trace<LDS_SCENE, WIDE>(sv, s_scene, s_stack, tid, kBlock, a.count != 0);
    if (!LDS_SCENE) __syncthreads();
    const int W = sv.cam.width;
    const double spp = (double)a.spp;
    AccLds acc; acc.slot = s_acc + tid; acc.stride = kBlock;
    acc.init();
    LanePriv lp; lp.slot = s_priv + tid; lp.stride = kBlock;
    LaneCounters lc = {0, 0, 0};
    TraceCounters tc = {0, 0, 0, 0, 0, 0};
    Lane L;
    Trav tv;
    trav_init(sv, tv, __builtin_huge_val());
    L.s = 0; L.s_end = 0; L.st = S_DONE;
    L.kc = 0; L.num_vertices = 0; L.mats = 0xFFFFFF; L.rng_state = 0; L.rng_inc = 1;
    L.org = L.dir = splat(0);
    int x = 0, y = 0;
    unsigned long long base = 0;
    long long my_item = -1;
    WaveQueue wq;
    __shared__ unsigned long long s_stamps[STAMPED ? (kBlock / 64) * (SEG_COUNT + 1) : 1];
    Stamps<STAMPED> stamps;
    stamps.start(s_stamps + (STAMPED ? (tid >> 6) * (SEG_COUNT + 1) : 0));
    unsigned long long t_dry = ~0ull;
    if (STAMPED && (tid & 63) == 0) atomicMin(&a.counters->stamps[SEG_T_START], __builtin_amdgcn_s_memrealtime());
    constexpr bool QUEUE_MID = LAMBERT;
    auto hand_out = [&](int &act) __attribute__((always_inline)) {
        const bool idle = (L.st == S_DONE);
        if (idle && my_item >= 0) {
            Accum r = acc.result();
            typedef double d2 __attribute__((ext_vector_type(2)));
            d2 *dst = (d2 *)(a.partials + (size_t)my_item * 16);
            dst[0] = d2{r.r.x, r.r.y}; dst[1] = d2{r.r.z, r.dx0.x}; dst[2] = d2{r.dx0.y, r.dx0.z}; dst[3] = d2{r.dy0.x, r.dy0.y};
            dst[4] = d2{r.dy0.z, r.dx1.x}; dst[5] = d2{r.dx1.y, r.dx1.z}; dst[6] = d2{r.dy1.x, r.dy1.y}; dst[7] = d2{r.dy1.z, 0.0};
            acc.init();
            my_item = -1;
        }
        stamps.mark(SEG_PUBLISH);
        const long long got_item = wq.take(a, idle, tid);
        stamps.mark(SEG_TAKE);
        if (STAMPED && wq.exhausted && t_dry == ~0ull) t_dry = __builtin_amdgcn_s_memrealtime();
        if (got_item >= 0) {
            my_item = got_item;
            int s0, s1;
            const bool inside = item_to_pixel(a, W, (unsigned)my_item, x, y, s0, s1, s_chunks);
            base = ((unsigned long long)y * W + x) * (unsigned long long)a.stream_spp;
            L.s = s0; L.s_end = s1;
            if (inside && s0 < s1) act = ACT_PRIMARY_RAY;
        }
        stamps.mark(SEG_ITEM);
    };
    for (;;) {
        int act = ACT_NONE;
        if (!QUEUE_MID) {
            hand_out(act);
            if (act == ACT_PRIMARY_RAY) L.st = S_START;
            if (!__any(L.st != S_DONE)) { if (wq.exhausted) break; else continue; }
            stamps.mark(SEG_QUEUE);
        }
        trace_pending<TraceCfg<WW, WIDE, !LDS_SCENE, !(PLAIN & kPlainNoSpheres), !LDS_SCENE>>(sv, tx, L, tv, a.thresh_a, a.thresh_c, tc);
        stamps.mark(SEG_TRACE);
        stamps.tick(SEG_STEPS);
        act = ACT_NONE;
        if (lane_ready(L, tv)) {
            if (tx.count) { tc.lane_steps++; if (wave_leader()) tc.wave_steps++; }
            act = lane_consume<LAMBERT, false, AccLds, Stamps<STAMPED>, PLAIN>(sv, tx, a.max_depth, spp, base, L, tv, lp, acc, lc, tc, &stamps);
        }
        if (QUEUE_MID) hand_out(act);
        lane_camera<false, Stamps<STAMPED>>(sv, act, x, y, base, L, tv, lp, &stamps);
        if (QUEUE_MID) {
            if (!__any(L.st != S_DONE) && wq.exhausted) break;
            stamps.mark(SEG_QUEUE);
        }
    }
    flush_counters(a, lc, tc, a.count != 0);
    if (STAMPED && (tid & 63) == 0) {
        for (int i = 0; i < SEG_COUNT; i++) atomicAdd(&a.counters->stamps[i], stamps.get(i));
        atomicMin(&a.counters->stamps[SEG_T_DRY], t_dry);
        atomicMax(&a.counters->stamps[SEG_T_END], __builtin_amdgcn_s_memrealtime());
    }
}

#ifdef GDPT_BUILD_REDUCE
__global__ __launch_bounds__(256) void gdpt_reduce_partials(KernelArgs a, int W) {
    const long long nslots = a.num_slots;
    const long long t = (long long)blockIdx.x * 256 + threadIdx.x;
    const long long idx = t >> 4;
    const int j = (int)(t & 15);
    if (idx >= nslots || j == 15) return;
    int x, y, s0, s1;
    if (!item_to_pixel(a, W, (unsigned)idx, x, y, s0, s1, a.chunk_begin)) return;
    const double *src = a.partials + (size_t)idx * 16 + j;
    double v = 0;
    for (int c = 0; c < a.num_chunks; c++) v += src[(size_t)c * (size_t)nslots * 16];
    double *img = (j < 3) ? a.img : (j < 6) ? a.cx0 : (j < 9) ? a.cy0 : (j < 12) ? a.cx1 : a.cy1;
    img[((size_t)y * W + x) * 3 + (j % 3)] = v;
}
#endif

template <bool LAMBERT>
__global__ __launch_bounds__(64) void gdpt_render_tile_stream_phases(DevSceneView sv, KernelArgs a, int ntx, int nty) {
    __shared__ int s_stack[GDPT_BVH_MAX_DEPTH * 64];
    __shared__ double s_priv[kPrivDoubles * 64];
    const int tid = threadIdx.x;
    const int tile = blockIdx.x * 64 + tid;
    TraceCtx tx = setup_trace<false, true>(sv, nullptr, s_stack, tid, 64, a.count != 0);
    LanePriv lp; lp.slot = s_priv + tid; lp.stride = 64;
    LaneCounters lc = {0, 0, 0};
    TraceCounters tc = {0, 0, 0, 0, 0, 0};
    const int W = sv.cam.width, H = sv.cam.height;
    const double spp = (double)a.spp;
    if (tile < ntx * nty) {
        const int txi = tile % ntx, tyi = tile / ntx;
        Lane L;
        { Pcg r0 = pcg_init((unsigned long long)(tyi * ntx + txi)); L.rng_state = r0.state; L.rng_inc = r0.inc; }
        L.kc = 0; L.num_vertices = 0; L.mats = 0xFFFFFF;
        L.org = L.dir = splat(0);
        Trav tv;
        trav_init(sv, tv, __builtin_huge_val());
        const int x0 = txi * 16, x1 = min(x0 + 16, W), y0 = tyi * 16, y1 = min(y0 + 16, H);
        for (int y = y0; y < y1; y++) {
            if (y < a.row_begin || y >= a.row_end) continue;
            for (int x = x0; x < x1; x++) {
                AccReg acc; acc.init();
                L.s = 0; L.s_end = a.spp; L.st = S_START;
                while (L.st != S_DONE) {
                    if (lane_tracing(L.st) && tv.cur != kTravDone)
                        trav_run<TraceHbm>(sv, tx, L.org, L.dir, (L.st == S_BOUNCE) ? (float)sv.isect_eps : 0.0f, __builtin_huge_valf(), tv, 0, 0, tc);
                    lane_step<LAMBERT, true>(sv, tx, a.max_depth, spp, x, y, 0ull, L, tv, lp, acc, lc, tc);
                }
                Accum sum = acc.result();
                reduce_and_store(a, sum, 1, true, x, y, W);
            }
        }
    }
    flush_counters(a, lc, tc, a.count != 0);
}

#ifdef GDPT_BUILD_EAGER
struct Offset { Vertex v; D3 dir; D3 contrib; double jacob; };
struct SampleOut { D3 radiance, contrib; D3 cX[4]; double w[4]; double prob; };

GD void zero_out(SampleOut &o) {
// ... 85 lines not shown
        }
        ray = bsdf_ray;
        vertex = bsdf_vertex;
        throughput = throughput * (G * f) / (p2 * rr_prob);
    }
    out.radiance = radiance; out.contrib = contrib; out.prob = prob;
    if (alive) {
#pragma unroll 1
        for (int k = 0; k < 4; k++)
            if (alive >> k & 1u) { out.cX[k] = off[k].contrib * off[k].jacob; out.w[k] = prob / (prob + 1.0 * off[k].jacob); }
    }
}

GD void accumulate_eager(AccReg &a, const SampleOut &s, double spp, LaneCounters &lc) {
    bool flagged = false;
#pragma unroll
    for (int k = 0; k < 4; k++) acc_offset(a, k, s.contrib, s.cX[k], s.w[k], s.prob, spp, lc, flagged);
    acc_base(a, s.radiance, s.prob, spp, lc, flagged);
}

__global__ __launch_bounds__(kBlock, 2) void gdpt_render_eager(DevSceneView sv, KernelArgs a) {
    __shared__ int s_stack[GDPT_BVH_MAX_DEPTH * kBlock];
    const int tid = threadIdx.x;
    TraceCtx tx = setup_trace<false, true>(sv, nullptr, s_stack, tid, kBlock, a.count != 0);
    const int K = 1 << a.log2k;
    const int c = tid & (K - 1), p = tid >> a.log2k;
    const int px = p % a.tile_w, py = p / a.tile_w;
    const int bx = blockIdx.x % a.tiles_x, by = blockIdx.x / a.tiles_x;
    const int x = bx * a.tile_w + px, y = a.row_begin + by * a.tile_h + py;
    const int W = sv.cam.width;
    const bool valid = (x < W) && (y < a.row_end);
    AccReg acc; acc.init();
    LaneCounters lc = {0, 0, 0};
    TraceCounters tc = {0, 0, 0, 0, 0, 0};
    if (valid) {
        const int s0 = (int)(((long long)c * a.spp) >> a.log2k), s1 = (int)(((long long)(c + 1) * a.spp) >> a.log2k);
        const unsigned long long base = ((unsigned long long)y * W + x) * (unsigned long long)a.stream_spp + (unsigned long long)a.first_sample;
        for (int s = s0; s < s1; s++) {
            Pcg rng = pcg_init(base + (unsigned long long)s);
            SampleOut so;
            grad_sample_eager(sv, tx, a.max_depth, x, y, rng, so, lc, tc);
            accumulate_eager(acc, so, (double)a.spp, lc);
        }
    }
    Accum sum = acc.result();
    reduce_and_store(a, sum, K, valid && c == 0, x, y, W);
    flush_counters(a, lc, tc, a.count != 0);
}

__global__ __launch_bounds__(64) void gdpt_render_tile_stream_eager(DevSceneView sv, KernelArgs a, int ntx, int nty) {
    __shared__ int s_stack[GDPT_BVH_MAX_DEPTH * 64];
    const int tid = threadIdx.x;
    const int tile = blockIdx.x * 64 + tid;
    TraceCtx tx = setup_trace<false, true>(sv, nullptr, s_stack, tid, 64, a.count != 0);
    LaneCounters lc = {0, 0, 0};
    TraceCounters tc = {0, 0, 0, 0, 0, 0};
    const int W = sv.cam.width, H = sv.cam.height;
    if (tile < ntx * nty) {
        const int txi = tile % ntx, tyi = tile / ntx;
        Pcg rng = pcg_init((unsigned long long)(tyi * ntx + txi));
        const int x0 = txi * 16, x1 = min(x0 + 16, W), y0 = tyi * 16, y1 = min(y0 + 16, H);
        for (int y = y0; y < y1; y++) {
            if (y < a.row_begin || y >= a.row_end) continue;
            for (int x = x0; x < x1; x++) {
                AccReg acc; acc.init();
                for (int s = 0; s < a.spp; s++) {
                    SampleOut so;
                    grad_sample_eager(sv, tx, a.max_depth, x, y, rng, so, lc, tc);
                    accumulate_eager(acc, so, (double)a.spp, lc);
                }
                Accum sum = acc.result();
                reduce_and_store(a, sum, 1, true, x, y, W);
            }
        }
    }
    flush_counters(a, lc, tc, a.count != 0);
}

#endif

}

namespace gdpt {
void launch_phases_lambert(const DevSceneView &sv, const gd::KernelArgs &a, dim3 grid, bool lds, bool lds_wide, hipStream_t stream);
void launch_phases_lambert_plain(const DevSceneView &sv, const gd::KernelArgs &a, dim3 grid, bool lds, bool const_tex, hipStream_t stream);
void launch_phases_lambert_stamped(const DevSceneView &sv, const gd::KernelArgs &a, dim3 grid, bool lds, bool plain, hipStream_t stream);
void launch_reduce_partials(const DevSceneView &sv, const gd::KernelArgs &a, hipStream_t stream);
void launch_phases_general(const DevSceneView &sv, const gd::KernelArgs &a, dim3 grid, bool lds, bool lds_wide, hipStream_t stream);
void launch_phases_general_set_a(const DevSceneView &sv, const gd::KernelArgs &a, dim3 grid, int lobe, hipStream_t stream);
void launch_phases_general_set_b(const DevSceneView &sv, const gd::KernelArgs &a, dim3 grid, int lobe, hipStream_t stream);
void launch_phases_twosided(const DevSceneView &sv, const gd::KernelArgs &a, dim3 grid, bool lds, void *bounce_log, hipStream_t stream);
void launch_phases_twosided_glass(const DevSceneView &sv, const gd::KernelArgs &a, dim3 grid, void *bounce_log, hipStream_t stream);
void launch_tile_phases_lambert(const DevSceneView &sv, const gd::KernelArgs &a, dim3 grid, int ntx, int nty, hipStream_t stream);
void launch_tile_phases_general(const DevSceneView &sv, const gd::KernelArgs &a, dim3 grid, int ntx, int nty, hipStream_t stream);
void launch_eager(const DevSceneView &sv, const gd::KernelArgs &a, dim3 grid, hipStream_t stream);
void launch_tile_eager(const DevSceneView &sv, const gd::KernelArgs &a, dim3 grid, int ntx, int nty, hipStream_t stream);
void launch_reconnect(const DevSceneView &sv, const gd::KernelArgs &a, dim3 grid, bool lds, bool lambert, hipStream_t stream);
void launch_path(const DevSceneView &sv, const gd::KernelArgs &a, dim3 grid, hipStream_t stream);
void launch_path_persistent(const DevSceneView &sv, const gd::KernelArgs &a, dim3 grid, bool lambert, bool lds, bool env, bool plain, hipStream_t stream);
void launch_tile_path(const DevSceneView &sv, const gd::KernelArgs &a, dim3 grid, int ntx, int nty, hipStream_t stream);
}
```

### gradient-based-path-tracing_amd/csrc/hip/render_kernels.h

```cpp
#pragma once
#include "../device_scene.h"
#include <hip/hip_runtime.h>

namespace gdpt {

constexpr int kMaxChunks = 64;
struct ChunkPlan { int n; int begin[kMaxChunks + 1]; };

struct RenderCounters {
    unsigned long long rays, bounces, nonfinite, nodes, prims;
    unsigned long long wave_node_trips, wave_leaf_trips, wave_steps, lane_steps;
    unsigned long long stamps[16];
};

enum class Route : int {
    LAMBERT_PLAIN_LDS_CONST, LAMBERT_PLAIN_LDS_TEX, LAMBERT_PLAIN_HBM_CONST, LAMBERT_PLAIN_HBM_TEX,
    LAMBERT_LDS_WIDE, LAMBERT_LDS_BVH2, LAMBERT_HBM,
    LAMBERT_STAMPED_LDS_PLAIN, LAMBERT_STAMPED_LDS, LAMBERT_STAMPED_HBM,
    GENERAL_SET_A_DISNEY_DIFFUSE, GENERAL_SET_A_DISNEY_METAL, GENERAL_SET_B_DISNEY_CLEARCOAT, GENERAL_SET_B_DISNEY_SHEEN,
    GENERAL_LDS_WIDE, GENERAL_LDS_BVH2, GENERAL_HBM,
    TWOSIDED_LDS, TWOSIDED_HBM, TWOSIDED_HBM_GLASS,
    WAVEFRONT_LAMBERT, WAVEFRONT_GENERAL,
    EAGER, TILE_EAGER, TILE_PHASES_LAMBERT, TILE_PHASES_GENERAL,
    RECONNECT_LDS_LAMBERT, RECONNECT_HBM_LAMBERT, RECONNECT_GENERAL,
    PATH_TILE, PATH_EAGER,
    PATH_PERSISTENT_LDS_LAMBERT_PLAIN, PATH_PERSISTENT_LDS_LAMBERT, PATH_PERSISTENT_LDS_LAMBERT_ENV,
    PATH_PERSISTENT_HBM_LAMBERT, PATH_PERSISTENT_HBM_LAMBERT_ENV,
    PATH_PERSISTENT_LDS_GENERAL, PATH_PERSISTENT_LDS_GENERAL_ENV, PATH_PERSISTENT_HBM_GENERAL, PATH_PERSISTENT_HBM_GENERAL_ENV,
    COUNT
};
const char *route_name(Route r);
inline bool is_path(Route r) { return r >= Route::PATH_TILE; }
inline bool is_persistent(Route r) { return r <= Route::WAVEFRONT_GENERAL || r >= Route::PATH_PERSISTENT_LDS_LAMBERT_PLAIN; }
inline bool is_wavefront(Route r) { return r == Route::WAVEFRONT_LAMBERT || r == Route::WAVEFRONT_GENERAL; }
inline bool needs_bounce_log(Route r) { return r >= Route::TWOSIDED_LDS && r <= Route::TWOSIDED_HBM_GLASS; }
inline bool is_stamped(Route r) { return r >= Route::LAMBERT_STAMPED_LDS_PLAIN && r <= Route::LAMBERT_STAMPED_HBM; }
inline bool can_overlap(Route r) { return r <= Route::GENERAL_HBM && !is_stamped(r); }
inline bool walks_bvh2(Route r) { return r == Route::LAMBERT_LDS_BVH2 || r == Route::GENERAL_LDS_BVH2; }

struct RouteInputs {
    bool path;
    int rng_scheme, shift_mode;
    int max_depth, rr_depth;
    bool one_sided;
    bool has_rough;
    bool lambert_only;
    unsigned material_mask;
    bool has_spheres, const_textures, has_envmap;
    bool fits_lds;
    bool fits_lds_wide;
    bool force_eager, no_lds_scene, lds_wide, no_twosided_machine, wavefront, stamps, no_plain_kernel, full_material_switch;
};
Route choose_route(const RouteInputs &in);

struct RenderLaunch {
    Route route;
    int spp;
    int stream_spp, first_sample;
    int row_begin, row_end;
    int max_depth;
    double *img, *cx0, *cy0, *cx1, *cy1;
    RenderCounters *counters;
    bool count_traversal;
    ChunkPlan plan;
    int thresh_a, thresh_c;
    int force_log2k;
    int wide_stack_need;
    void *bounce_log;
    size_t bounce_log_bytes;
    int num_cus;
    int blocks_per_cu;
    unsigned long long *wf_state;
    unsigned *wf_live;
    void *wf_aux;
    int wf_sort;
    float wf_bounds[6];
    unsigned *wf_counters;
    unsigned *wf_host;
    hipEvent_t wf_event;
    int wf_slots;
    int replay_per_step;
    double *partials;
    unsigned long long *queue_head;
    hipStream_t kernel_stream;
    hipEvent_t kernel_done;
};
bool scene_fits_lds(int num_nodes, int num_prims, int num_tris, int num_materials, int num_lights, int bvh_depth);
bool scene_fits_lds_wide(int num_nodes4, int num_prims, int num_tris, int num_materials, int num_lights, int wide_stack_need);

inline long long resident_lanes(const RenderLaunch &rl) { return (long long)rl.num_cus * (rl.blocks_per_cu > 0 ? rl.blocks_per_cu : 2) * 256; }
inline long long band_slots(int width, int rows) { return (long long)((width + 15) / 16) * ((rows + 15) / 16) * 256; }
size_t twosided_log_bytes(unsigned blocks);
unsigned persistent_blocks(const RenderLaunch &rl, long long num_items);
ChunkPlan make_chunk_plan(int spp, int force_log2k, long long pixels, long long lanes, int take_pct = 0);

int wf_words();
int wf_max_generations();
int wf_slot_count(long long num_items);
size_t wf_aux_bytes(int slots);
void launch_render(const DevSceneView &sv, const RenderLaunch &rl, hipStream_t stream);

void set_route(Route r);
void reset_route();
const char *last_route();
int route_names(const char **out, int capacity);
bool twosided_log_covers(int max_depth, int rr_depth);

}
```

### gradient-based-path-tracing_amd/csrc/hip/render_kernels.hip

```cpp
#include "render_twosided.h"
#include "render_wavefront.h"

#include "../capi_common.h"
#include <stdexcept>
#include <string>

namespace gdpt {

namespace {
thread_local const char *g_route = "";
const char *const kRouteNames[] = {
    "lambert_plain/lds_const", "lambert_plain/lds_tex", "lambert_plain/hbm_const", "lambert_plain/hbm_tex",
    "lambert/lds_wide", "lambert/lds_bvh2", "lambert/hbm",
    "lambert_stamped/lds_plain", "lambert_stamped/lds", "lambert_stamped/hbm",
    "general_set_a/disney_diffuse", "general_set_a/disney_metal", "general_set_b/disney_clearcoat", "general_set_b/disney_sheen",
    "general/lds_wide", "general/lds_bvh2", "general/hbm",
    "twosided/lds", "twosided/hbm", "twosided/hbm_glass",
    "wavefront/lambert", "wavefront/general",
    "eager", "tile_eager", "tile_phases_lambert", "tile_phases_general",
    "reconnect/lds_lambert", "reconnect/hbm_lambert", "reconnect/general",
    "path/tile", "path/eager",
    "path_persistent/lds_lambert_plain", "path_persistent/lds_lambert", "path_persistent/lds_lambert_env",
    "path_persistent/hbm_lambert", "path_persistent/hbm_lambert_env",
    "path_persistent/lds_general", "path_persistent/lds_general_env", "path_persistent/hbm_general", "path_persistent/hbm_general_env",
// ... 103 lines not shown
    l.hist = take((size_t)gd::kWfBins * 4); l.offsets = take((size_t)gd::kWfBins * 4);
    l.blocks = take((size_t)(slots / gd::kBlock) * 16);
    l.ovf = take((size_t)slots * (size_t)(GDPT_BVH_MAX_DEPTH - gd::kWfLdsLevels) * 4);
    l.total = off;
    return l;
}
}
size_t wf_aux_bytes(int slots) { return wf_aux_layout(slots).total; }

static void run_wavefront(const DevSceneView &sv, const gd::KernelArgs &a, const RenderLaunch &rl, bool lambert, hipStream_t stream) {
    static_assert(GDPT_BVH_MAX_DEPTH > gd::kWfLdsLevels, "overflow stack levels");
    const WfAux lay = wf_aux_layout(rl.wf_slots);
    char *aux = (char *)rl.wf_aux;
    gd::WfBuf w{};
    w.state = rl.wf_state; w.live = rl.wf_live; w.counters = rl.wf_counters; w.n = rl.wf_slots; w.gen = 0;
    w.rays = (float4 *)(aux + lay.rays); w.hits = (float4 *)(aux + lay.hits); w.keys = (uint2 *)(aux + lay.keys);
    w.hist = (unsigned *)(aux + lay.hist); w.offsets = (unsigned *)(aux + lay.offsets);
    w.block_counts = (uint4 *)(aux + lay.blocks); w.totals = rl.counters;
    w.sort = rl.wf_sort; w.tiles_x = (sv.cam.width + 15) / 16;
    for (int k = 0; k < 3; k++) {
        const float lo = rl.wf_bounds[k], hi = rl.wf_bounds[3 + k];
        w.bmin[k] = lo;
        w.cell_scale[k] = (hi > lo) ? 16.0f / (hi - lo) : 0.0f;
    }
    gd::WfTrace t{};
    t.nodes4 = sv.nodes4; t.nodes4q = sv.nodes4q; t.prims = sv.prims; t.spheres = sv.spheres; t.rays = w.rays; t.hits = w.hits; t.live = w.live;
    t.ovf = (int *)(aux + lay.ovf); t.ovf_stride = (unsigned)rl.wf_slots; t.counters = rl.counters;
    t.num_tris = sv.num_tris; t.num_nodes4 = sv.num_nodes4; t.num_spheres = sv.num_spheres; t.search_frac = a.thresh_c; t.count_stats = a.count;
    auto ckh = [](hipError_t e, const char *what) { if (e != hipSuccess) throw std::runtime_error(std::string(what) + ": " + hipGetErrorString(e)); };
    ckh(hipMemsetAsync(rl.wf_counters, 0, sizeof(unsigned) * 3 * gd::kWfMaxGen, stream), "hipMemsetAsync(wavefront counters)");
    ckh(hipMemsetAsync(w.hist, 0, sizeof(unsigned) * gd::kWfBins, stream), "hipMemsetAsync(wavefront histogram)");
    launch_wf_init(w, stream);
    unsigned active_bound = (unsigned)rl.wf_slots;
    const int chunk = 8;
    int gen = 0;
    auto enqueue_chunk = [&]() {
        for (int k = 0; k < chunk; k++, gen++) {
            if (gen >= gd::kWfMaxGen) throw std::runtime_error("launch_render: wavefront generation limit reached");
            w.gen = gen;
            if (lambert) launch_wf_step_lambert(sv, a, w, stream); else launch_wf_step_general(sv, a, w, stream);
            launch_wf_sort(w, stream);
            t.count = rl.wf_counters + gen;
            launch_wf_trace(t, sv.num_spheres > 0, (active_bound + gd::kWfTraceBlock - 1) / gd::kWfTraceBlock, stream);
        }
    };
    enqueue_chunk();
    for (;;) {
        ckh(hipMemcpyAsync(rl.wf_host, rl.wf_counters + 2 * gd::kWfMaxGen + (gen - 1), sizeof(unsigned), hipMemcpyDeviceToHost, stream), "hipMemcpyAsync(wavefront live count)");
        ckh(hipEventRecord(rl.wf_event, stream), "hipEventRecord");
        const bool room = gen + chunk <= gd::kWfMaxGen;
        if (room) enqueue_chunk();
        ckh(hipEventSynchronize(rl.wf_event), "hipEventSynchronize");
        if (*rl.wf_host == 0u) break;
        if (*rl.wf_host < active_bound) active_bound = *rl.wf_host;
        if (!room) throw std::runtime_error("launch_render: wavefront generation limit reached");
    }
}

void launch_render(const DevSceneView &sv, const RenderLaunch &rl, hipStream_t stream) {
    const Route r = rl.route;
    if (rl.kernel_stream && (!can_overlap(r) || !rl.kernel_done)) throw std::runtime_error("launch_render: this route does not overlap");
    const hipStream_t ks = rl.kernel_stream ? rl.kernel_stream : stream;
    gd::KernelArgs a{};
    a.spp = rl.spp; a.stream_spp = rl.stream_spp; a.first_sample = rl.first_sample; a.row_begin = rl.row_begin; a.row_end = rl.row_end; a.max_depth = rl.max_depth;
    a.img = rl.img; a.cx0 = rl.cx0; a.cy0 = rl.cy0; a.cx1 = rl.cx1; a.cy1 = rl.cy1; a.counters = rl.counters;
    a.thresh_a = rl.thresh_a >= 0 ? (rl.thresh_a > 255 ? 255 : rl.thresh_a) : 64;
    a.thresh_c = rl.thresh_c >= 0 ? (rl.thresh_c > 255 ? 255 : rl.thresh_c) : 112;
    a.count = rl.count_traversal ? 1 : 0;
    const int W = sv.cam.width, rows = rl.row_end - rl.row_begin;
    if (W <= 0 || rows <= 0 || rl.spp <= 0) throw std::runtime_error("launch_render: empty image band or spp <= 0");
    if (rl.first_sample < 0 || (long long)rl.first_sample + rl.spp > (long long)rl.stream_spp) throw std::runtime_error("launch_render: sample window outside its stream block");
    const int ntx = (W + 15) / 16, nty = (sv.cam.height + 15) / 16;
    dim3 grid((unsigned)((ntx * nty + 63) / 64));
    if (is_persistent(r)) {
        a.stack_levels = rl.wide_stack_need > 0 ? rl.wide_stack_need : GDPT_BVH_MAX_DEPTH;
        a.replay_per_step = rl.replay_per_step >= 1 ? rl.replay_per_step : 4;
        if (a.stack_levels > GDPT_BVH_MAX_DEPTH) throw std::runtime_error("launch_render: traversal stack bound exceeds the builder's maximum");
        grid = start_queue(a, rl, W, ks);
    }
    if (needs_bounce_log(r) && (!rl.bounce_log || rl.bounce_log_bytes < twosided_log_bytes(grid.x))) throw std::runtime_error("launch_render: bounce log missing");
    if (is_wavefront(r) && (!rl.wf_state || !rl.wf_live || !rl.wf_counters || !rl.wf_host || !rl.wf_aux || rl.wf_slots <= 0))
        throw std::runtime_error("launch_render: wavefront buffers missing");
    set_route(r);
    switch (r) {
    case Route::LAMBERT_PLAIN_LDS_CONST: launch_phases_lambert_plain(sv, a, grid, true, true, ks); break;
    case Route::LAMBERT_PLAIN_LDS_TEX: launch_phases_lambert_plain(sv, a, grid, true, false, ks); break;
    case Route::LAMBERT_PLAIN_HBM_CONST: launch_phases_lambert_plain(sv, a, grid, false, true, ks); break;
    case Route::LAMBERT_PLAIN_HBM_TEX: launch_phases_lambert_plain(sv, a, grid, false, false, ks); break;
    case Route::LAMBERT_LDS_WIDE: launch_phases_lambert(sv, a, grid, true, true, ks); break;
    case Route::LAMBERT_LDS_BVH2: launch_phases_lambert(sv, a, grid, true, false, ks); break;
    case Route::LAMBERT_HBM: launch_phases_lambert(sv, a, grid, false, false, ks); break;
    case Route::LAMBERT_STAMPED_LDS_PLAIN: launch_phases_lambert_stamped(sv, a, grid, true, true, stream); break;
    case Route::LAMBERT_STAMPED_LDS: launch_phases_lambert_stamped(sv, a, grid, true, false, stream); break;
    case Route::LAMBERT_STAMPED_HBM: launch_phases_lambert_stamped(sv, a, grid, false, false, stream); break;
    case Route::GENERAL_SET_A_DISNEY_DIFFUSE: launch_phases_general_set_a(sv, a, grid, GDPT_MAT_DISNEY_DIFFUSE, ks); break;
    case Route::GENERAL_SET_A_DISNEY_METAL: launch_phases_general_set_a(sv, a, grid, GDPT_MAT_DISNEY_METAL, ks); break;
    case Route::GENERAL_SET_B_DISNEY_CLEARCOAT: launch_phases_general_set_b(sv, a, grid, GDPT_MAT_DISNEY_CLEARCOAT, ks); break;
    case Route::GENERAL_SET_B_DISNEY_SHEEN: launch_phases_general_set_b(sv, a, grid, GDPT_MAT_DISNEY_SHEEN, ks); break;
    case Route::GENERAL_LDS_WIDE: launch_phases_general(sv, a, grid, true, true, ks); break;
    case Route::GENERAL_LDS_BVH2: launch_phases_general(sv, a, grid, true, false, ks); break;
    case Route::GENERAL_HBM: launch_phases_general(sv, a, grid, false, false, ks); break;
    case Route::TWOSIDED_LDS: launch_phases_twosided(sv, a, grid, true, rl.bounce_log, stream); break;
    case Route::TWOSIDED_HBM: launch_phases_twosided(sv, a, grid, false, rl.bounce_log, stream); break;
    case Route::TWOSIDED_HBM_GLASS: launch_phases_twosided_glass(sv, a, grid, rl.bounce_log, stream); break;
    case Route::WAVEFRONT_LAMBERT: run_wavefront(sv, a, rl, true, stream); break;
    case Route::WAVEFRONT_GENERAL: run_wavefront(sv, a, rl, false, stream); break;
    case Route::EAGER: launch_eager(sv, a, static_mapping(a, rl, W, rows), stream); break;
    case Route::TILE_EAGER: launch_tile_eager(sv, a, grid, ntx, nty, stream); break;
    case Route::TILE_PHASES_LAMBERT: launch_tile_phases_lambert(sv, a, grid, ntx, nty, stream); break;
    case Route::TILE_PHASES_GENERAL: launch_tile_phases_general(sv, a, grid, ntx, nty, stream); break;
    case Route::RECONNECT_LDS_LAMBERT: launch_reconnect(sv, a, static_mapping(a, rl, W, rows), true, true, stream); break;
    case Route::RECONNECT_HBM_LAMBERT: launch_reconnect(sv, a, static_mapping(a, rl, W, rows), false, true, stream); break;
    case Route::RECONNECT_GENERAL: launch_reconnect(sv, a, static_mapping(a, rl, W, rows), false, false, stream); break;
    case Route::PATH_TILE: launch_tile_path(sv, a, grid, ntx, nty, stream); break;
    case Route::PATH_EAGER: launch_path(sv, a, static_mapping(a, rl, W, rows), stream); break;
    case Route::PATH_PERSISTENT_LDS_LAMBERT_PLAIN: launch_path_persistent(sv, a, grid, true, true, false, true, stream); break;
    case Route::PATH_PERSISTENT_LDS_LAMBERT: launch_path_persistent(sv, a, grid, true, true, false, false, stream); break;
    case Route::PATH_PERSISTENT_LDS_LAMBERT_ENV: launch_path_persistent(sv, a, grid, true, true, true, false, stream); break;
    case Route::PATH_PERSISTENT_HBM_LAMBERT: launch_path_persistent(sv, a, grid, true, false, false, false, stream); break;
    case Route::PATH_PERSISTENT_HBM_LAMBERT_ENV: launch_path_persistent(sv, a, grid, true, false, true, false, stream); break;
    case Route::PATH_PERSISTENT_LDS_GENERAL: launch_path_persistent(sv, a, grid, false, true, false, false, stream); break;
    case Route::PATH_PERSISTENT_LDS_GENERAL_ENV: launch_path_persistent(sv, a, grid, false, true, true, false, stream); break;
    case Route::PATH_PERSISTENT_HBM_GENERAL: launch_path_persistent(sv, a, grid, false, false, false, false, stream); break;
    case Route::PATH_PERSISTENT_HBM_GENERAL_ENV: launch_path_persistent(sv, a, grid, false, false, true, false, stream); break;
    case Route::COUNT: throw std::runtime_error("launch_render: no route");
    }
    if (rl.kernel_stream) {
        if (hipEventRecord(rl.kernel_done, ks) != hipSuccess || hipStreamWaitEvent(stream, rl.kernel_done, 0) != hipSuccess)
            throw std::runtime_error("launch_render: joining the render stream failed");
    }
    if (is_persistent(r) && !is_path(r)) launch_reduce_partials(sv, a, stream);
    hipError_t e = hipGetLastError();
    if (e != hipSuccess) throw std::runtime_error(std::string("render kernel launch failed: ") + hipGetErrorString(e));
}

unsigned persistent_blocks(const RenderLaunch &rl, long long num_items) {
    long long waves_needed = (num_items + 63) / 64;
    long long blocks = resident_lanes(rl) / gd::kBlock;
    if (blocks > (waves_needed + 3) / 4) blocks = (waves_needed + 3) / 4;
    return (unsigned)(blocks < 1 ? 1 : blocks);
}

ChunkPlan make_chunk_plan(int spp, int force_log2k, long long pixels, long long lanes, int take_pct_arg) {
    ChunkPlan p{};
    if (spp < 1) spp = 1;
    if (force_log2k >= 0) {
        int k = force_log2k;
        while (k > 0 && ((1 << k) > spp || (1 << k) > kMaxChunks)) k--;
        p.n = 1 << k;
        for (int c = 0; c <= p.n; c++) p.begin[c] = (int)(((long long)c * spp) >> k);
        return p;
    }
    {
        long long digits = (long long)gdpt::debug_knob("plan_digits", 0.0);
        int sz[18], m = 0, sum = 0;
        for (; digits > 0 && m < 18; digits /= 10) { sz[m] = (int)(digits % 10); sum += sz[m]; if (sz[m] == 0) sum = -1000000; m++; }
        if (m > 0 && sum == spp) {
            p.n = m; p.begin[0] = 0;
            for (int c = 0; c < m; c++) p.begin[c + 1] = p.begin[c] + sz[m - 1 - c];
            return p;
        }
    }
    long long cap = (long long)spp * pixels / (lanes > 0 ? lanes * 4 : 1);
    if (cap < 1) cap = 1;
    long long rounds = gdpt::debug_knob_int("plan_rounds", 4);
    rounds = rounds <= 0 ? 4 : std::min(8LL, rounds);
    long long q = (pixels > 0 && rounds * lanes > pixels) ? (rounds * lanes + pixels - 1) / pixels : 1;
    if (q > 8) q = 8;
    if ((long long)spp <= q) q = 1;
    const long long slots = kMaxChunks / q;
    const long long head = q > 1 ? (slots > 4 ? slots - 4 : 1) : kMaxChunks - 8;
    const int v = (int)(((long long)spp + q - 1) / q);
    if ((long long)v > cap * head) cap = ((long long)v + head - 1) / head;
    long long take_pct = gdpt::debug_knob_int("plan_shrink", 0);
    if (take_pct <= 0) take_pct = take_pct_arg > 0 ? take_pct_arg : 55;
    take_pct = std::min(90LL, std::max(10LL, take_pct));
    int sizes[kMaxChunks];
    int rem = v, m = 0;
    while (rem > 0) {
        long long sz = ((long long)rem * take_pct + 99) / 100;
        if (rem <= 2) sz = 1;
        if (sz > cap) sz = cap;
        if (sz < 1) sz = 1;
        if (m == (int)slots - 1) sz = rem;
// ... 34 lines not shown
```

### gradient-based-path-tracing_amd/csrc/hip/render_phases_diag.hip

```cpp
#include "render_device.h"
namespace gdpt {
void launch_phases_lambert_stamped(const DevSceneView &sv, const gd::KernelArgs &a, dim3 grid, bool lds, bool plain, hipStream_t stream) {
    if (lds && plain) hipLaunchKernelGGL((gd::gdpt_render_phases<true, true, true, true, true, gd::kPlainBoth>), grid, dim3(gd::kBlock), 0, stream, sv, a);
    else if (lds) hipLaunchKernelGGL((gd::gdpt_render_phases<true, true, true, true, true>), grid, dim3(gd::kBlock), 0, stream, sv, a);
    else hipLaunchKernelGGL((gd::gdpt_render_phases<true, false, true, true, true>), grid, dim3(gd::kBlock), gd::hbm_dynamic_lds(a), stream, sv, a);
}
}
```

### gradient-based-path-tracing_amd/csrc/hip/render_phases_general.hip

```cpp
#include "render_device.h"
namespace gdpt {
void launch_phases_general(const DevSceneView &sv, const gd::KernelArgs &a, dim3 grid, bool lds, bool lds_wide, hipStream_t stream) {
    if (lds && lds_wide) hipLaunchKernelGGL((gd::gdpt_render_phases<false, true, true, true>), grid, dim3(gd::kBlock), 0, stream, sv, a);
    else if (lds) hipLaunchKernelGGL((gd::gdpt_render_phases<false, true, false, false>), grid, dim3(gd::kBlock), 0, stream, sv, a);
    else hipLaunchKernelGGL((gd::gdpt_render_phases<false, false, true, true>), grid, dim3(gd::kBlock), gd::hbm_dynamic_lds(a), stream, sv, a);
}
void launch_tile_phases_general(const DevSceneView &sv, const gd::KernelArgs &a, dim3 grid, int ntx, int nty, hipStream_t stream) {
    hipLaunchKernelGGL((gd::gdpt_render_tile_stream_phases<false>), grid, dim3(64), 0, stream, sv, a, ntx, nty);
}
}
```

### gradient-based-path-tracing_amd/csrc/hip/render_phases_lambert.hip

```cpp
#define GDPT_BUILD_REDUCE 1
#include "render_device.h"
namespace gdpt {
void launch_phases_lambert(const DevSceneView &sv, const gd::KernelArgs &a, dim3 grid, bool lds, bool lds_wide, hipStream_t stream) {
    if (lds && lds_wide) hipLaunchKernelGGL((gd::gdpt_render_phases<true, true, true, true>), grid, dim3(gd::kBlock), 0, stream, sv, a);
    else if (lds) hipLaunchKernelGGL((gd::gdpt_render_phases<true, true, false, false>), grid, dim3(gd::kBlock), 0, stream, sv, a);
    else hipLaunchKernelGGL((gd::gdpt_render_phases<true, false, true, true>), grid, dim3(gd::kBlock), gd::hbm_dynamic_lds(a), stream, sv, a);
}
void launch_reduce_partials(const DevSceneView &sv, const gd::KernelArgs &a, hipStream_t stream) {
    const long long nslots = a.num_slots;
    hipLaunchKernelGGL(gd::gdpt_reduce_partials, dim3((unsigned)((nslots * 16 + 255) / 256)), dim3(256), 0, stream, a, sv.cam.width);
}
void launch_tile_phases_lambert(const DevSceneView &sv, const gd::KernelArgs &a, dim3 grid, int ntx, int nty, hipStream_t stream) {
    hipLaunchKernelGGL((gd::gdpt_render_tile_stream_phases<true>), grid, dim3(64), 0, stream, sv, a, ntx, nty);
}
}
```

### gradient-based-path-tracing_amd/csrc/hip/render_phases_lambert_plain.hip

```cpp
#include "render_device.h"
namespace gdpt {
void launch_phases_lambert_plain(const DevSceneView &sv, const gd::KernelArgs &a, dim3 grid, bool lds, bool const_tex, hipStream_t stream) {
    if (lds && const_tex) hipLaunchKernelGGL((gd::gdpt_render_phases<true, true, true, true, false, gd::kPlainBoth>), grid, dim3(gd::kBlock), 0, stream, sv, a);
    else if (lds) hipLaunchKernelGGL((gd::gdpt_render_phases<true, true, true, true, false, gd::kPlainNoSpheres>), grid, dim3(gd::kBlock), 0, stream, sv, a);
    else if (const_tex) hipLaunchKernelGGL((gd::gdpt_render_phases<true, false, true, true, false, gd::kPlainBoth>), grid, dim3(gd::kBlock), gd::hbm_dynamic_lds(a), stream, sv, a);
    else hipLaunchKernelGGL((gd::gdpt_render_phases<true, false, true, true, false, gd::kPlainNoSpheres>), grid, dim3(gd::kBlock), gd::hbm_dynamic_lds(a), stream, sv, a);
}
}
```

### gradient-based-path-tracing_amd/csrc/hip/scene_internal.h

```cpp
#pragma once
#include "../../../include/gdpt.h"
#include "../device_scene.h"
#include "device_mem.h"
#include "render_kernels.h"

#include <hip/hip_runtime.h>

#include <stdexcept>
#include <string>
#include <vector>

struct GdptLaunchScratch {
    gdpt::DeviceBuffer<double> partials;
    gdpt::DeviceBuffer<unsigned long long> queue;
    gdpt::DeviceBuffer<gdpt::RenderCounters> counters;
    gdpt::Event rendered;
    gdpt::Event released;
    bool used = false;
};

struct GdptScene {
    int device = 0;
    DevSceneView view{};
    int bvh_depth = 0;
    int wide_stack_need = 0;
    int wide8_stack_need = 0;
    bool has_envmap = false;
    int scene_spp = 0;
    bool one_sided = true, lambert_only = true;
    unsigned material_mask = 0;
    int plan_take_pct = 0;
    bool has_rough = false;
    std::vector<gdpt::DeviceBuffer<unsigned char>> allocations;
    gdpt::DeviceBuffer<double> d_buf[9];
    gdpt::RenderCounters *d_counters = nullptr;
    gdpt::PinnedBuffer<gdpt::RenderCounters> h_counters;
    gdpt::DeviceBuffer<unsigned char> d_bounce_log;
    GdptLaunchScratch scratch[2];
    gdpt::Stream render_stream[2];
    gdpt::Event ev_entry[2];
    unsigned long long calls = 0;
    unsigned long long overlapped = 0;
    bool in_flight = false;
    bool need_fence = true;
    bool have_caller = false;
    hipStream_t last_caller = nullptr;
    gdpt::DeviceBuffer<unsigned long long> d_wf_state;
    gdpt::DeviceBuffer<unsigned> d_wf_live, d_wf_counters;
    gdpt::PinnedBuffer<unsigned> h_wf_word;
    gdpt::DeviceBuffer<unsigned char> d_wf_aux;
    float bounds[6] = {0, 0, 0, 0, 0, 0};
    gdpt::Event wf_event;
    int num_cus = 256;
    gdpt::Event ev0, ev1;

    void ensure_buffers(size_t elems) {
        for (auto &b : d_buf) b.grow(elems, "hipMalloc(image buffers)");
    }
    void join() {
        if (!in_flight) return;
        for (auto &st : render_stream) if (st) gdpt::ck(hipStreamSynchronize(st), "hipStreamSynchronize(render stream)");
        in_flight = false;
    }
    ~GdptScene() {
        hipSetDevice(device);
        for (auto &st : render_stream) st.reset();
        for (auto &ss : scratch) if (ss.used) (void)hipEventSynchronize(ss.released);
    }
};


namespace gdpt {
void build_scene(const GdptSceneDesc *desc, int device, GdptScene *sc);
void render_device_impl(GdptScene *sc, const GdptRenderParams *params, int scene_spp,
                        double *img, double *cx0, double *cy0, double *cx1, double *cy1,
                        hipStream_t stream, GdptRenderStats *stats, const GdptSampleWindow *window = nullptr);
}
```

### include/gdpt_debug.h

```cpp
#ifndef GDPT_DEBUG_H
#define GDPT_DEBUG_H
#include <stdint.h>
#ifdef __cplusplus
extern "C" {
#endif

int gdpt_debug_knob_set(const char *name, double value);
void gdpt_debug_get_stamps(double out[16]);
int gdpt_debug_chunk_plan(int spp, int force_log2k, long long film_pixels, long long resident_lanes, int32_t *begin, int capacity);
const char *gdpt_debug_last_route(void);
struct GdptScene;
long long gdpt_debug_overlapped_launches(const struct GdptScene *scene);
int gdpt_debug_route_names(const char **out, int capacity);
void gdpt_debug_knobs_reset(void);

#ifdef __cplusplus
}
#endif
#endif
```

Measured before the change: 2012.

## Split LDS-scene BVH leaf tests into two-primitive steps interleaved with traversal

```diff
diff --git a/gradient-based-path-tracing_amd/__init__.py b/gradient-based-path-tracing_amd/__init__.py
--- a/gradient-based-path-tracing_amd/__init__.py
+++ b/gradient-based-path-tracing_amd/__init__.py
@@ -113,6 +113,7 @@
         L.gdpt_debug_last_route.restype = C.c_char_p
         L.gdpt_debug_overlapped_launches.argtypes = [vp]
         L.gdpt_debug_overlapped_launches.restype = C.c_longlong
+        L.gdpt_debug_leaf_histogram.argtypes = [vp, C.POINTER(C.c_int32)]
         L.gdpt_debug_route_names.argtypes = [C.POINTER(C.c_char_p), C.c_int]
         _LIB = L
     return _LIB
@@ -250,6 +251,11 @@
         _check(lib().gdpt_tile_row_costs(self.handle, int(spp), buf, T))
         return [float(x) for x in buf]
 
+    def leaf_histogram(self):
+        h = (C.c_int32 * 4)()
+        _check(lib().gdpt_debug_leaf_histogram(self.handle, h))
+        return list(h)
+
     def overlapped_launches(self):
         return int(lib().gdpt_debug_overlapped_launches(self.handle))
 
@@ -762,7 +768,7 @@
     def from_env(environ=None):
         environ = os.environ if environ is None else environ
         names = ("force_eager", "log2k", "keep_frac", "search_frac", "blocks_per_cu", "no_lds_scene", "lds_wide",
-                 "no_twosided_machine", "presplit", "presplit_floor", "bvh_leaf_max", "bvh_leaf_factor", "sbvh", "sbvh_alpha", "plan_rounds", "plan_shrink", "plan_digits", "bvh_collapse_dp", "stamps", "wavefront", "wf_slots", "wf_sort", "multi_fail_band", "multi_fail_stage", "dct_bk", "dct_bm", "full_material_switch", "no_plain_kernel", "replay_per_step", "no_render_overlap")
+                 "no_twosided_machine", "presplit", "presplit_floor", "bvh_leaf_max", "bvh_leaf_factor", "sbvh", "sbvh_alpha", "plan_rounds", "plan_shrink", "plan_digits", "bvh_collapse_dp", "stamps", "wavefront", "wf_slots", "wf_sort", "multi_fail_band", "multi_fail_stage", "dct_bk", "dct_bm", "full_material_switch", "no_plain_kernel", "replay_per_step", "no_render_overlap", "whole_leaf_trips")
         lib().gdpt_debug_knobs_reset()
         for n in names:
             v = environ.get("GDPT_" + n.upper())
diff --git a/gradient-based-path-tracing_amd/csrc/capi_host.cpp b/gradient-based-path-tracing_amd/csrc/capi_host.cpp
--- a/gradient-based-path-tracing_amd/csrc/capi_host.cpp
+++ b/gradient-based-path-tracing_amd/csrc/capi_host.cpp
@@ -24,7 +24,7 @@
 std::mutex g_knob_mu;
 std::map<std::string, double> g_knobs;
 const char *const kKnobNames[] = {"force_eager", "log2k", "keep_frac", "search_frac", "blocks_per_cu", "no_lds_scene", "lds_wide",
-                                  "no_twosided_machine", "presplit", "presplit_floor", "bvh_leaf_max", "bvh_leaf_factor", "sbvh", "sbvh_alpha", "plan_rounds", "plan_shrink", "plan_digits", "bvh_collapse_dp", "stamps", "wavefront", "wf_slots", "wf_sort", "multi_fail_band", "multi_fail_stage", "dct_bk", "dct_bm", "full_material_switch", "no_plain_kernel", "replay_per_step", "no_render_overlap"};
+                                  "no_twosided_machine", "presplit", "presplit_floor", "bvh_leaf_max", "bvh_leaf_factor", "sbvh", "sbvh_alpha", "plan_rounds", "plan_shrink", "plan_digits", "bvh_collapse_dp", "stamps", "wavefront", "wf_slots", "wf_sort", "multi_fail_band", "multi_fail_stage", "dct_bk", "dct_bm", "full_material_switch", "no_plain_kernel", "replay_per_step", "no_render_overlap", "whole_leaf_trips"};
 double g_stamps[16] = {0};
 }
 void debug_store_stamps(const unsigned long long *v, int n) {
diff --git a/gradient-based-path-tracing_amd/csrc/device_scene.h b/gradient-based-path-tracing_amd/csrc/device_scene.h
--- a/gradient-based-path-tracing_amd/csrc/device_scene.h
+++ b/gradient-based-path-tracing_amd/csrc/device_scene.h
@@ -48,6 +48,12 @@
 };
 #ifndef GDPT_HBM_Q4
 #define GDPT_HBM_Q4 1
+#endif
+#ifndef GDPT_LDS_LEAF_K
+#define GDPT_LDS_LEAF_K 2
+#endif
+#ifndef GDPT_LDS_LEAF_FLAT
+#define GDPT_LDS_LEAF_FLAT 1
 #endif
 
 struct DevPrim {
diff --git a/gradient-based-path-tracing_amd/csrc/hip/capi_device.hip b/gradient-based-path-tracing_amd/csrc/hip/capi_device.hip
--- a/gradient-based-path-tracing_amd/csrc/hip/capi_device.hip
+++ b/gradient-based-path-tracing_amd/csrc/hip/capi_device.hip
@@ -160,6 +160,8 @@
     std::vector<DevPrim> prims(bvh.order.size());
     for (size_t i = 0; i < bvh.order.size(); i++) prims[i] = prim_in[ref_prim[bvh.order[i]]];
     sc->bvh_depth = bvh.depth;
+    for (const DevBvhNode &n : bvh.nodes)
+        for (int32_t ch : {n.left, n.right}) if (ch < 0 && ch != GDPT_CHILD_EMPTY) sc->leaf_hist[~(unsigned)ch & 3u]++;
     if (bvh.depth > GDPT_BVH_MAX_DEPTH) throw std::runtime_error("gdpt_scene_upload: BVH deeper than the traversal stack (builder bug)");
 
     std::vector<DevImage> images;
@@ -486,9 +488,10 @@
     in.force_eager = knob("force_eager", 0) != 0; in.no_lds_scene = knob("no_lds_scene", 0) != 0; in.lds_wide = knob("lds_wide", 1) != 0;
     in.no_twosided_machine = knob("no_twosided_machine", 0) != 0; in.wavefront = knob("wavefront", kWavefrontDefault) != 0;
     in.stamps = knob("stamps", 0) != 0; in.no_plain_kernel = knob("no_plain_kernel", 0) != 0;
-    in.full_material_switch = knob("full_material_switch", 0) != 0;
+    in.full_material_switch = knob("full_material_switch", 0) != 0; in.whole_leaf_trips = knob("whole_leaf_trips", 0) != 0;
     gdpt::RenderLaunch rl{};
     rl.route = gdpt::choose_route(in);
+    rl.whole_leaf_trips = in.whole_leaf_trips;
     rl.spp = b.spp; rl.stream_spp = b.stream_spp; rl.first_sample = b.first_sample; rl.row_begin = b.row_begin; rl.row_end = b.row_end; rl.max_depth = b.max_depth;
     rl.count_traversal = stats && stats->nodes_visited == ~0ull;
     rl.force_log2k = knob("log2k", -1);
@@ -672,6 +675,12 @@
 
 const char *gdpt_debug_last_route(void) { return gdpt::last_route(); }
 long long gdpt_debug_overlapped_launches(const GdptScene *scene) { return scene ? (long long)scene->overlapped : -1; }
+int gdpt_debug_leaf_histogram(const GdptScene *scene, int32_t hist[4]) {
+    return gdpt::guarded([&]() {
+        if (!scene || !hist) throw std::runtime_error("gdpt_debug_leaf_histogram: null argument");
+        for (int i = 0; i < 4; i++) hist[i] = scene->leaf_hist[i];
+    });
+}
 int gdpt_debug_route_names(const char **out, int capacity) { return gdpt::route_names(out, capacity); }
 
 int gdpt_scene_upload(const GdptSceneDesc *desc, int device, GdptScene **out_scene) {
diff --git a/gradient-based-path-tracing_amd/csrc/hip/render_device.h b/gradient-based-path-tracing_amd/csrc/hip/render_device.h
--- a/gradient-based-path-tracing_amd/csrc/hip/render_device.h
+++ b/gradient-based-path-tracing_amd/csrc/hip/render_device.h
@@ -1,6 +1,7 @@
 #pragma once
 #include "render_kernels.h"
 #include "device_trace.h"
+#include "../leaf_cursor.h"
 
 namespace gd {
 
@@ -266,6 +267,25 @@
         test_tri_flat(p2, o, d, tnear, tfar, last >= 2u, best);
         test_tri_flat(p3, o, d, tnear, tfar, last >= 3u, best);
     }
+}
+
+template <int K, bool FLAT, bool SPHERES = true>
+GD bool leaf_step(const DevSceneView &sv, const TraceCtx &tx, int &cur, const float o[3], const float d[3], float tnear, float tfar,
+                  Hit &best, TraceCounters &tc) {
+    static_assert(K == 1 || K == 2, "leaf_step: one or two records per step");
+    const unsigned packed = ~(unsigned)cur;
+    const unsigned first = packed >> 2, last = packed & 3u;
+    const DevPrim p0 = tx.prims[first];
+    const DevPrim p1 = tx.prims[first + (K > 1 ? min(1u, last) : 0u)];
+    if (tx.count) { tc.prims += leaf_step_records(cur, K); if (wave_leader()) tc.leaf_trips++; }
+    if (!FLAT || (SPHERES && ((p0.gid | p1.gid) & GDPT_SPHERE_FLAG))) {
+        test_prim<SPHERES>(sv, p0, o, d, tnear, tfar, best);
+        if (K > 1 && last >= 1u) test_prim<SPHERES>(sv, p1, o, d, tnear, tfar, best);
+    } else {
+        test_tri_flat(p0, o, d, tnear, tfar, true, best);
+        if (K > 1) test_tri_flat(p1, o, d, tnear, tfar, last >= 1u, best);
+    }
+    return !leaf_advance(cur, K);
 }
 
 constexpr int kTravDone = INT32_MIN;
@@ -345,7 +365,11 @@
         else trav_pop(tx, cur, sp);
     }
 }
-template <bool WW_, bool WIDE_, bool FLAT_, bool SPHERES_ = true, bool SPEC_ = false> struct TraceCfg { static constexpr bool WW = WW_, WIDE = WIDE_, FLAT = FLAT_, SPHERES = SPHERES_, SPEC = SPEC_ || GDPT_SPEC_LEAF; };
+template <bool WW_, bool WIDE_, bool FLAT_, bool SPHERES_ = true, bool SPEC_ = false, int LEAF_K_ = 0> struct TraceCfg {
+    static constexpr bool WW = WW_, WIDE = WIDE_, FLAT = FLAT_, SPHERES = SPHERES_, SPEC = SPEC_ || GDPT_SPEC_LEAF;
+    static constexpr int LEAF_K = LEAF_K_;
+    static constexpr bool LEAF_FLAT = FLAT_ || GDPT_LDS_LEAF_FLAT;
+};
 using TraceHbm = TraceCfg<true, true, true>;
 
 template <class TC>
@@ -366,6 +390,7 @@
         if (TC::WW) {
             const int few = (live * search_frac) >> 8;
             if (TC::SPEC) {
+                static_assert(!(TC::SPEC && TC::LEAF_K > 0), "the speculative leaf hold takes whole leaves");
                 int held = kTravDone;
                 for (;;) {
                     if (cur < 0 && cur != kTravDone && held == kTravDone) { held = cur; trav_pop<kOvf>(tx, cur, sp, tv.ovf); }
@@ -390,8 +415,12 @@
                     }
                 }
                 if (cur < 0 && cur != kTravDone) {
-                    test_leaf<TC::FLAT, TC::SPHERES>(sv, tx, cur, o, d, tnear, tfar, best, tc);
-                    trav_pop<kOvf>(tx, cur, sp, tv.ovf);
+                    if constexpr (TC::LEAF_K > 0) {
+                        if (leaf_step<TC::LEAF_K, TC::LEAF_FLAT, TC::SPHERES>(sv, tx, cur, o, d, tnear, tfar, best, tc)) trav_pop<kOvf>(tx, cur, sp, tv.ovf);
+                    } else {
+                        test_leaf<TC::FLAT, TC::SPHERES>(sv, tx, cur, o, d, tnear, tfar, best, tc);
+                        trav_pop<kOvf>(tx, cur, sp, tv.ovf);
+                    }
                     if (any_hit && best.gid >= 0) cur = kTravDone;
                 }
             }
@@ -399,8 +428,12 @@
             if (tx.count) { tc.nodes++; if (wave_leader()) tc.node_trips++; }
             trav_node<TC::WIDE, TC::FLAT>(tx, oi, inv, tnear, best.t, cur, sp, tv.ovf);
         } else if (cur != kTravDone) {
-            test_leaf<TC::FLAT, TC::SPHERES>(sv, tx, cur, o, d, tnear, tfar, best, tc);
-            trav_pop<kOvf>(tx, cur, sp, tv.ovf);
+            if constexpr (TC::LEAF_K > 0) {
+                if (leaf_step<TC::LEAF_K, TC::LEAF_FLAT, TC::SPHERES>(sv, tx, cur, o, d, tnear, tfar, best, tc)) trav_pop<kOvf>(tx, cur, sp, tv.ovf);
+            } else {
+                test_leaf<TC::FLAT, TC::SPHERES>(sv, tx, cur, o, d, tnear, tfar, best, tc);
+                trav_pop<kOvf>(tx, cur, sp, tv.ovf);
+            }
             if (any_hit && best.gid >= 0) cur = kTravDone;
         }
     }
@@ -799,7 +832,7 @@
     }
 };
 
-template <bool LAMBERT, bool LDS_SCENE, bool WIDE, bool WW, bool STAMPED = false, int PLAIN = 0>
+template <bool LAMBERT, bool LDS_SCENE, bool WIDE, bool WW, bool STAMPED = false, int PLAIN = 0, int LEAF_K = (LDS_SCENE && !GDPT_SPEC_LEAF ? GDPT_LDS_LEAF_K : 0)>
 __global__ __launch_bounds__(kBlock, 2) void gdpt_render_phases(DevSceneView sv, KernelArgs a) {
     __shared__ int s_stack_fixed[LDS_SCENE ? kLdsSceneLevels * kBlock : 1];
     __shared__ __attribute__((aligned(16))) unsigned char s_scene[LDS_SCENE ? kLdsSceneBytes : 16];
@@ -868,7 +901,7 @@
             if (!__any(L.st != S_DONE)) { if (wq.exhausted) break; else continue; }
             stamps.mark(SEG_QUEUE);
         }
-        trace_pending<TraceCfg<WW, WIDE, !LDS_SCENE, !(PLAIN & kPlainNoSpheres), !LDS_SCENE>>(sv, tx, L, tv, a.thresh_a, a.thresh_c, tc);
+        trace_pending<TraceCfg<WW, WIDE, !LDS_SCENE, !(PLAIN & kPlainNoSpheres), !LDS_SCENE, LEAF_K>>(sv, tx, L, tv, a.thresh_a, a.thresh_c, tc);
         stamps.mark(SEG_TRACE);
         stamps.tick(SEG_STEPS);
         act = ACT_NONE;
@@ -1120,11 +1153,11 @@
 }
 
 namespace gdpt {
-void launch_phases_lambert(const DevSceneView &sv, const gd::KernelArgs &a, dim3 grid, bool lds, bool lds_wide, hipStream_t stream);
-void launch_phases_lambert_plain(const DevSceneView &sv, const gd::KernelArgs &a, dim3 grid, bool lds, bool const_tex, hipStream_t stream);
-void launch_phases_lambert_stamped(const DevSceneView &sv, const gd::KernelArgs &a, dim3 grid, bool lds, bool plain, hipStream_t stream);
+void launch_phases_lambert(const DevSceneView &sv, const gd::KernelArgs &a, dim3 grid, bool lds, bool lds_wide, bool whole_leaf, hipStream_t stream);
+void launch_phases_lambert_plain(const DevSceneView &sv, const gd::KernelArgs &a, dim3 grid, bool lds, bool const_tex, bool whole_leaf, hipStream_t stream);
+void launch_phases_lambert_stamped(const DevSceneView &sv, const gd::KernelArgs &a, dim3 grid, bool lds, bool plain, bool whole_leaf, hipStream_t stream);
 void launch_reduce_partials(const DevSceneView &sv, const gd::KernelArgs &a, hipStream_t stream);
-void launch_phases_general(const DevSceneView &sv, const gd::KernelArgs &a, dim3 grid, bool lds, bool lds_wide, hipStream_t stream);
+void launch_phases_general(const DevSceneView &sv, const gd::KernelArgs &a, dim3 grid, bool lds, bool lds_wide, bool whole_leaf, hipStream_t stream);
 void launch_phases_general_set_a(const DevSceneView &sv, const gd::KernelArgs &a, dim3 grid, int lobe, hipStream_t stream);
 void launch_phases_general_set_b(const DevSceneView &sv, const gd::KernelArgs &a, dim3 grid, int lobe, hipStream_t stream);
 void launch_phases_twosided(const DevSceneView &sv, const gd::KernelArgs &a, dim3 grid, bool lds, void *bounce_log, hipStream_t stream);
diff --git a/gradient-based-path-tracing_amd/csrc/hip/render_kernels.h b/gradient-based-path-tracing_amd/csrc/hip/render_kernels.h
--- a/gradient-based-path-tracing_amd/csrc/hip/render_kernels.h
+++ b/gradient-based-path-tracing_amd/csrc/hip/render_kernels.h
@@ -50,6 +50,7 @@
     bool fits_lds;
     bool fits_lds_wide;
     bool force_eager, no_lds_scene, lds_wide, no_twosided_machine, wavefront, stamps, no_plain_kernel, full_material_switch;
+    bool whole_leaf_trips;
 };
 Route choose_route(const RouteInputs &in);
 
@@ -80,6 +81,7 @@
     hipEvent_t wf_event;
     int wf_slots;
     int replay_per_step;
+    bool whole_leaf_trips;
     double *partials;
     unsigned long long *queue_head;
     hipStream_t kernel_stream;
diff --git a/gradient-based-path-tracing_amd/csrc/hip/render_kernels.hip b/gradient-based-path-tracing_amd/csrc/hip/render_kernels.hip
--- a/gradient-based-path-tracing_amd/csrc/hip/render_kernels.hip
+++ b/gradient-based-path-tracing_amd/csrc/hip/render_kernels.hip
@@ -209,24 +209,25 @@
     if (is_wavefront(r) && (!rl.wf_state || !rl.wf_live || !rl.wf_counters || !rl.wf_host || !rl.wf_aux || rl.wf_slots <= 0))
         throw std::runtime_error("launch_render: wavefront buffers missing");
     set_route(r);
+    const bool wl = rl.whole_leaf_trips;
     switch (r) {
-    case Route::LAMBERT_PLAIN_LDS_CONST: launch_phases_lambert_plain(sv, a, grid, true, true, ks); break;
-    case Route::LAMBERT_PLAIN_LDS_TEX: launch_phases_lambert_plain(sv, a, grid, true, false, ks); break;
-    case Route::LAMBERT_PLAIN_HBM_CONST: launch_phases_lambert_plain(sv, a, grid, false, true, ks); break;
-    case Route::LAMBERT_PLAIN_HBM_TEX: launch_phases_lambert_plain(sv, a, grid, false, false, ks); break;
-    case Route::LAMBERT_LDS_WIDE: launch_phases_lambert(sv, a, grid, true, true, ks); break;
-    case Route::LAMBERT_LDS_BVH2: launch_phases_lambert(sv, a, grid, true, false, ks); break;
-    case Route::LAMBERT_HBM: launch_phases_lambert(sv, a, grid, false, false, ks); break;
-    case Route::LAMBERT_STAMPED_LDS_PLAIN: launch_phases_lambert_stamped(sv, a, grid, true, true, stream); break;
-    case Route::LAMBERT_STAMPED_LDS: launch_phases_lambert_stamped(sv, a, grid, true, false, stream); break;
-    case Route::LAMBERT_STAMPED_HBM: launch_phases_lambert_stamped(sv, a, grid, false, false, stream); break;
+    case Route::LAMBERT_PLAIN_LDS_CONST: launch_phases_lambert_plain(sv, a, grid, true, true, wl, ks); break;
+    case Route::LAMBERT_PLAIN_LDS_TEX: launch_phases_lambert_plain(sv, a, grid, true, false, wl, ks); break;
+    case Route::LAMBERT_PLAIN_HBM_CONST: launch_phases_lambert_plain(sv, a, grid, false, true, wl, ks); break;
+    case Route::LAMBERT_PLAIN_HBM_TEX: launch_phases_lambert_plain(sv, a, grid, false, false, wl, ks); break;
+    case Route::LAMBERT_LDS_WIDE: launch_phases_lambert(sv, a, grid, true, true, wl, ks); break;
+    case Route::LAMBERT_LDS_BVH2: launch_phases_lambert(sv, a, grid, true, false, wl, ks); break;
+    case Route::LAMBERT_HBM: launch_phases_lambert(sv, a, grid, false, false, wl, ks); break;
+    case Route::LAMBERT_STAMPED_LDS_PLAIN: launch_phases_lambert_stamped(sv, a, grid, true, true, wl, stream); break;
+    case Route::LAMBERT_STAMPED_LDS: launch_phases_lambert_stamped(sv, a, grid, true, false, wl, stream); break;
+    case Route::LAMBERT_STAMPED_HBM: launch_phases_lambert_stamped(sv, a, grid, false, false, wl, stream); break;
     case Route::GENERAL_SET_A_DISNEY_DIFFUSE: launch_phases_general_set_a(sv, a, grid, GDPT_MAT_DISNEY_DIFFUSE, ks); break;
     case Route::GENERAL_SET_A_DISNEY_METAL: launch_phases_general_set_a(sv, a, grid, GDPT_MAT_DISNEY_METAL, ks); break;
     case Route::GENERAL_SET_B_DISNEY_CLEARCOAT: launch_phases_general_set_b(sv, a, grid, GDPT_MAT_DISNEY_CLEARCOAT, ks); break;
     case Route::GENERAL_SET_B_DISNEY_SHEEN: launch_phases_general_set_b(sv, a, grid, GDPT_MAT_DISNEY_SHEEN, ks); break;
-    case Route::GENERAL_LDS_WIDE: launch_phases_general(sv, a, grid, true, true, ks); break;
-    case Route::GENERAL_LDS_BVH2: launch_phases_general(sv, a, grid, true, false, ks); break;
-    case Route::GENERAL_HBM: launch_phases_general(sv, a, grid, false, false, ks); break;
+    case Route::GENERAL_LDS_WIDE: launch_phases_general(sv, a, grid, true, true, wl, ks); break;
+    case Route::GENERAL_LDS_BVH2: launch_phases_general(sv, a, grid, true, false, wl, ks); break;
+    case Route::GENERAL_HBM: launch_phases_general(sv, a, grid, false, false, wl, ks); break;
     case Route::TWOSIDED_LDS: launch_phases_twosided(sv, a, grid, true, rl.bounce_log, stream); break;
     case Route::TWOSIDED_HBM: launch_phases_twosided(sv, a, grid, false, rl.bounce_log, stream); break;
     case Route::TWOSIDED_HBM_GLASS: launch_phases_twosided_glass(sv, a, grid, rl.bounce_log, stream); break;
diff --git a/gradient-based-path-tracing_amd/csrc/hip/render_phases_diag.hip b/gradient-based-path-tracing_amd/csrc/hip/render_phases_diag.hip
--- a/gradient-based-path-tracing_amd/csrc/hip/render_phases_diag.hip
+++ b/gradient-based-path-tracing_amd/csrc/hip/render_phases_diag.hip
@@ -1,7 +1,9 @@
 #include "render_device.h"
 namespace gdpt {
-void launch_phases_lambert_stamped(const DevSceneView &sv, const gd::KernelArgs &a, dim3 grid, bool lds, bool plain, hipStream_t stream) {
-    if (lds && plain) hipLaunchKernelGGL((gd::gdpt_render_phases<true, true, true, true, true, gd::kPlainBoth>), grid, dim3(gd::kBlock), 0, stream, sv, a);
+void launch_phases_lambert_stamped(const DevSceneView &sv, const gd::KernelArgs &a, dim3 grid, bool lds, bool plain, bool whole_leaf, hipStream_t stream) {
+    if (lds && plain && whole_leaf) hipLaunchKernelGGL((gd::gdpt_render_phases<true, true, true, true, true, gd::kPlainBoth, 0>), grid, dim3(gd::kBlock), 0, stream, sv, a);
+    else if (lds && plain) hipLaunchKernelGGL((gd::gdpt_render_phases<true, true, true, true, true, gd::kPlainBoth>), grid, dim3(gd::kBlock), 0, stream, sv, a);
+    else if (lds && whole_leaf) hipLaunchKernelGGL((gd::gdpt_render_phases<true, true, true, true, true, 0, 0>), grid, dim3(gd::kBlock), 0, stream, sv, a);
     else if (lds) hipLaunchKernelGGL((gd::gdpt_render_phases<true, true, true, true, true>), grid, dim3(gd::kBlock), 0, stream, sv, a);
     else hipLaunchKernelGGL((gd::gdpt_render_phases<true, false, true, true, true>), grid, dim3(gd::kBlock), gd::hbm_dynamic_lds(a), stream, sv, a);
 }
diff --git a/gradient-based-path-tracing_amd/csrc/hip/render_phases_general.hip b/gradient-based-path-tracing_amd/csrc/hip/render_phases_general.hip
--- a/gradient-based-path-tracing_amd/csrc/hip/render_phases_general.hip
+++ b/gradient-based-path-tracing_amd/csrc/hip/render_phases_general.hip
@@ -1,7 +1,9 @@
 #include "render_device.h"
 namespace gdpt {
-void launch_phases_general(const DevSceneView &sv, const gd::KernelArgs &a, dim3 grid, bool lds, bool lds_wide, hipStream_t stream) {
-    if (lds && lds_wide) hipLaunchKernelGGL((gd::gdpt_render_phases<false, true, true, true>), grid, dim3(gd::kBlock), 0, stream, sv, a);
+void launch_phases_general(const DevSceneView &sv, const gd::KernelArgs &a, dim3 grid, bool lds, bool lds_wide, bool whole_leaf, hipStream_t stream) {
+    if (lds && lds_wide && whole_leaf) hipLaunchKernelGGL((gd::gdpt_render_phases<false, true, true, true, false, 0, 0>), grid, dim3(gd::kBlock), 0, stream, sv, a);
+    else if (lds && lds_wide) hipLaunchKernelGGL((gd::gdpt_render_phases<false, true, true, true>), grid, dim3(gd::kBlock), 0, stream, sv, a);
+    else if (lds && whole_leaf) hipLaunchKernelGGL((gd::gdpt_render_phases<false, true, false, false, false, 0, 0>), grid, dim3(gd::kBlock), 0, stream, sv, a);
     else if (lds) hipLaunchKernelGGL((gd::gdpt_render_phases<false, true, false, false>), grid, dim3(gd::kBlock), 0, stream, sv, a);
     else hipLaunchKernelGGL((gd::gdpt_render_phases<false, false, true, true>), grid, dim3(gd::kBlock), gd::hbm_dynamic_lds(a), stream, sv, a);
 }
diff --git a/gradient-based-path-tracing_amd/csrc/hip/render_phases_lambert.hip b/gradient-based-path-tracing_amd/csrc/hip/render_phases_lambert.hip
--- a/gradient-based-path-tracing_amd/csrc/hip/render_phases_lambert.hip
+++ b/gradient-based-path-tracing_amd/csrc/hip/render_phases_lambert.hip
@@ -1,8 +1,10 @@
 #define GDPT_BUILD_REDUCE 1
 #include "render_device.h"
 namespace gdpt {
-void launch_phases_lambert(const DevSceneView &sv, const gd::KernelArgs &a, dim3 grid, bool lds, bool lds_wide, hipStream_t stream) {
-    if (lds && lds_wide) hipLaunchKernelGGL((gd::gdpt_render_phases<true, true, true, true>), grid, dim3(gd::kBlock), 0, stream, sv, a);
+void launch_phases_lambert(const DevSceneView &sv, const gd::KernelArgs &a, dim3 grid, bool lds, bool lds_wide, bool whole_leaf, hipStream_t stream) {
+    if (lds && lds_wide && whole_leaf) hipLaunchKernelGGL((gd::gdpt_render_phases<true, true, true, true, false, 0, 0>), grid, dim3(gd::kBlock), 0, stream, sv, a);
+    else if (lds && lds_wide) hipLaunchKernelGGL((gd::gdpt_render_phases<true, true, true, true>), grid, dim3(gd::kBlock), 0, stream, sv, a);
+    else if (lds && whole_leaf) hipLaunchKernelGGL((gd::gdpt_render_phases<true, true, false, false, false, 0, 0>), grid, dim3(gd::kBlock), 0, stream, sv, a);
     else if (lds) hipLaunchKernelGGL((gd::gdpt_render_phases<true, true, false, false>), grid, dim3(gd::kBlock), 0, stream, sv, a);
     else hipLaunchKernelGGL((gd::gdpt_render_phases<true, false, true, true>), grid, dim3(gd::kBlock), gd::hbm_dynamic_lds(a), stream, sv, a);
 }
diff --git a/gradient-based-path-tracing_amd/csrc/hip/render_phases_lambert_plain.hip b/gradient-based-path-tracing_amd/csrc/hip/render_phases_lambert_plain.hip
--- a/gradient-based-path-tracing_amd/csrc/hip/render_phases_lambert_plain.hip
+++ b/gradient-based-path-tracing_amd/csrc/hip/render_phases_lambert_plain.hip
@@ -1,7 +1,9 @@
 #include "render_device.h"
 namespace gdpt {
-void launch_phases_lambert_plain(const DevSceneView &sv, const gd::KernelArgs &a, dim3 grid, bool lds, bool const_tex, hipStream_t stream) {
-    if (lds && const_tex) hipLaunchKernelGGL((gd::gdpt_render_phases<true, true, true, true, false, gd::kPlainBoth>), grid, dim3(gd::kBlock), 0, stream, sv, a);
+void launch_phases_lambert_plain(const DevSceneView &sv, const gd::KernelArgs &a, dim3 grid, bool lds, bool const_tex, bool whole_leaf, hipStream_t stream) {
+    if (lds && const_tex && whole_leaf) hipLaunchKernelGGL((gd::gdpt_render_phases<true, true, true, true, false, gd::kPlainBoth, 0>), grid, dim3(gd::kBlock), 0, stream, sv, a);
+    else if (lds && const_tex) hipLaunchKernelGGL((gd::gdpt_render_phases<true, true, true, true, false, gd::kPlainBoth>), grid, dim3(gd::kBlock), 0, stream, sv, a);
+    else if (lds && whole_leaf) hipLaunchKernelGGL((gd::gdpt_render_phases<true, true, true, true, false, gd::kPlainNoSpheres, 0>), grid, dim3(gd::kBlock), 0, stream, sv, a);
     else if (lds) hipLaunchKernelGGL((gd::gdpt_render_phases<true, true, true, true, false, gd::kPlainNoSpheres>), grid, dim3(gd::kBlock), 0, stream, sv, a);
     else if (const_tex) hipLaunchKernelGGL((gd::gdpt_render_phases<true, false, true, true, false, gd::kPlainBoth>), grid, dim3(gd::kBlock), gd::hbm_dynamic_lds(a), stream, sv, a);
     else hipLaunchKernelGGL((gd::gdpt_render_phases<true, false, true, true, false, gd::kPlainNoSpheres>), grid, dim3(gd::kBlock), gd::hbm_dynamic_lds(a), stream, sv, a);
diff --git a/gradient-based-path-tracing_amd/csrc/hip/scene_internal.h b/gradient-based-path-tracing_amd/csrc/hip/scene_internal.h
--- a/gradient-based-path-tracing_amd/csrc/hip/scene_internal.h
+++ b/gradient-based-path-tracing_amd/csrc/hip/scene_internal.h
@@ -23,6 +23,7 @@
     int device = 0;
     DevSceneView view{};
     int bvh_depth = 0;
+    int leaf_hist[4] = {0, 0, 0, 0};
     int wide_stack_need = 0;
     int wide8_stack_need = 0;
     bool has_envmap = false;
diff --git a/gradient-based-path-tracing_amd/csrc/leaf_cursor.h b/gradient-based-path-tracing_amd/csrc/leaf_cursor.h
--- /dev/null
+++ b/gradient-based-path-tracing_amd/csrc/leaf_cursor.h
@@ -0,0 +1,23 @@
+#pragma once
+
+#if defined(__HIPCC__)
+#define GDPT_LEAF_HD __host__ __device__ inline
+#else
+#define GDPT_LEAF_HD inline
+#endif
+
+namespace gd {
+
+GDPT_LEAF_HD unsigned leaf_step_records(int cur, int K) {
+    const unsigned count = (~(unsigned)cur & 3u) + 1u;
+    return count < (unsigned)K ? count : (unsigned)K;
+}
+
+GDPT_LEAF_HD bool leaf_advance(int &cur, int K) {
+    const unsigned packed = ~(unsigned)cur;
+    if ((packed & 3u) < (unsigned)K) return false;
+    cur = (int)~(packed + 3u * (unsigned)K);
+    return true;
+}
+
+}
diff --git a/include/gdpt_debug.h b/include/gdpt_debug.h
--- a/include/gdpt_debug.h
+++ b/include/gdpt_debug.h
@@ -11,6 +11,7 @@
 const char *gdpt_debug_last_route(void);
 struct GdptScene;
 long long gdpt_debug_overlapped_launches(const struct GdptScene *scene);
+int gdpt_debug_leaf_histogram(const struct GdptScene *scene, int32_t hist[4]);
 int gdpt_debug_route_names(const char **out, int capacity);
 void gdpt_debug_knobs_reset(void);
 
```

Result: faster. 2119 (median of 6 runs) (+5.3%).
